# QinLab-WFU/CLIP-based-Cross-Modal-Hashing

Measured on AMD Instinct MI355X. Metric: image+text pairs/s encoded+hashed per GPU; mAP@K eval wallclock (64-bit), higher is better.
Workload: dtype bf16

## Files before the change

### clip-based-cross-modal-hashing_amd/csrc/gemm_lc.hip

```cpp
#include <cstdlib>
#include <cstring>

#include "cmh_common.h"

#include <hip/hip_ext.h>

namespace cmh {

typedef __attribute__((ext_vector_type(8))) __bf16 lc_bf16x8_t;
typedef __attribute__((ext_vector_type(4))) float lc_f32x4_t;
typedef __attribute__((ext_vector_type(2))) float lc_f32x2_t;
typedef __attribute__((ext_vector_type(4))) uint32_t lc_u32x4_t;
typedef __attribute__((ext_vector_type(2))) unsigned lc_u2_t;
typedef const __attribute__((address_space(1))) void* lc_gptr_t;
typedef __attribute__((address_space(3))) void* lc_lptr_t;

constexpr int lcBM = 128, lcBN = 256;
constexpr int lcRowBytes = 128;
constexpr int lcWBytes = lcBN * lcRowBytes;
constexpr int lcSTG = lcWBytes + lcBM * lcRowBytes;

struct LcProblem {
  const char* X; const char* W; const float* bias; const void* residual; void* out;
  const int* m_dev;
  int Mub, N, K;
  const float* colscale = nullptr;
  float alpha = 1.f, oscale = 1.f;
};

__device__ __forceinline__ int lc_swz(int row, int chunk) { return row * lcRowBytes + ((chunk ^ (row & 7)) << 4); }

#define LC_READ(dst, addr, off) asm volatile("ds_read_b128 %0, %1 offset:" #off : "=v"(dst) : "v"(addr))

#ifdef LC_STAMPS
__device__ unsigned long long g_lc_stamps[256 * 8];
#define LC_T() __builtin_amdgcn_s_memtime()
#endif

template <bool GRP, int RES, bool F16O, int ABL = 0>
__global__ __launch_bounds__(512) void gemm_lc_kernel(LcProblem p0, LcProblem p1, int epi) {
  constexpr bool RF = RES == 1;
  __shared__ __attribute__((aligned(1024))) char lds[3 * lcSTG + 2 * 1024];
  const int tid = threadIdx.x;
  const int lane = tid & 63;
  const int wid = __builtin_amdgcn_readfirstlane(tid >> 6);

  const char* const X0 = p0.X; const char* const W0 = p0.W; const float* const B0 = p0.bias;
  const void* const R0 = p0.residual; void* const O0 = p0.out;
  const int N0 = p0.N, K0 = p0.K;
  const char* const X1 = p1.X; const char* const W1 = p1.W; const float* const B1 = p1.bias;
  const void* const R1 = p1.residual; void* const O1 = p1.out;
  const int N1 = p1.N, K1 = p1.K;
  int M0 = p0.Mub;
  if (p0.m_dev) { const int md = *p0.m_dev; M0 = md < M0 ? md : M0; }
  M0 = __builtin_amdgcn_readfirstlane(M0);
  int M1 = 0;
  if constexpr (GRP) {
    M1 = p1.Mub;
    if (p1.m_dev) { const int md = *p1.m_dev; M1 = md < M1 ? md : M1; }
    M1 = __builtin_amdgcn_readfirstlane(M1);
  }
  const int tiles_n0 = N0 / lcBN, tiles_n1 = GRP ? N1 / lcBN : 1;
  const int total0 = tiles_n0 * ((M0 + lcBM - 1) / lcBM);
  const int total1 = GRP ? tiles_n1 * ((M1 + lcBM - 1) / lcBM) : 0;
  const int xcd = blockIdx.x & 7, slot = blockIdx.x >> 3, per = gridDim.x >> 3;
  const int q0 = total0 >> 3, r0 = total0 & 7, q1 = total1 >> 3, r1 = total1 & 7;
  const int lo0 = xcd < r0 ? xcd * (q0 + 1) : r0 * (q0 + 1) + (xcd - r0) * q0, len0 = xcd < r0 ? q0 + 1 : q0;
  const int lo1 = xcd < r1 ? xcd * (q1 + 1) : r1 * (q1 + 1) + (xcd - r1) * q1, len1 = xcd < r1 ? q1 + 1 : q1;
  const int n_first = slot < len0 ? (len0 - slot + per - 1) / per : 0;
  const int span = len0 + len1;
  const int my_tiles = slot < span ? (span - slot + per - 1) / per : 0;
  if (my_tiles == 0) return;
  const int nk0 = K0 / 64, nk1 = GRP ? K1 / 64 : 0;
  const int S = n_first * nk0 + (my_tiles - n_first) * nk1;
  auto tile_of = [&](int ti, bool& second, int& m0, int& n0) {
    const int j = slot + ti * per;
    second = GRP && ti >= n_first;
    const int logical = second ? lo1 + (j - len0) : lo0 + j;
    const int tn_cnt = second ? tiles_n1 : tiles_n0;
    const int tm = logical / tn_cnt;
    m0 = tm * lcBM;
    n0 = (logical - tm * tn_cnt) * lcBN;
  };

  if (wid < 4) {
    const int sub = lane >> 3, ch = lane & 7;
    uint32_t offW[8], offX[4];
    const char* Wt = nullptr;
    const char* Xt = nullptr;
    const char* Bt = nullptr;
    int i_nk = 0;
    int w_prob = -1;
    auto set_tile = [&](int ti) {
      bool second; int m0, n0;
      tile_of(ti, second, m0, n0);
      const uint32_t rs = static_cast<uint32_t>(second ? K1 : K0) * 2;
      if (w_prob != static_cast<int>(second)) {
        w_prob = static_cast<int>(second);
#pragma unroll
        for (int i = 0; i < 8; ++i) {
          const int row = (wid * 8 + i) * 8 + sub;
          offW[i] = static_cast<uint32_t>(row) * rs + ((ch ^ (row & 7)) << 4);
        }
      }
      i_nk = second ? nk1 : nk0;
      const int Mp = second ? M1 : M0;
      Wt = (second ? W1 : W0) + static_cast<size_t>(n0) * rs;
      Xt = second ? X1 : X0;
      Bt = reinterpret_cast<const char*>((second ? B1 : B0) + n0);
#pragma unroll
      for (int i = 0; i < 4; ++i) {
        const int row = (wid * 4 + i) * 8 + sub;
        int xr = m0 + row;
        xr = xr < Mp ? xr : Mp - 1;
        offX[i] = static_cast<uint32_t>(xr) * rs + ((ch ^ (row & 7)) << 4);
      }
    };
    int i_tile = 0, i_kt = 0, ibuf = 0;
    set_tile(0);
    const bool bias_wave = wid == 0 && (epi & EPI_BIAS);
    auto issue_stage = [&]() {
      char* base = lds + ibuf * lcSTG;
      const uint32_t koff = static_cast<uint32_t>(i_kt) * lcRowBytes;
      if (i_kt == 0 && bias_wave)
        __builtin_amdgcn_global_load_lds((lc_gptr_t)(Bt + lane * 16), (lc_lptr_t)(lds + 3 * lcSTG + (i_tile & 1) * 1024), 16, 0, 0);
#pragma unroll
      for (int i = 0; i < 8; ++i)
        __builtin_amdgcn_global_load_lds((lc_gptr_t)(Wt + koff + offW[i]), (lc_lptr_t)(base + (wid * 8 + i) * 1024), 16, 0, 0);
#pragma unroll
      for (int i = 0; i < 4; ++i)
        __builtin_amdgcn_global_load_lds((lc_gptr_t)(Xt + koff + offX[i]), (lc_lptr_t)(base + lcWBytes + (wid * 4 + i) * 1024), 16, 0, 0);
      ibuf = ibuf == 2 ? 0 : ibuf + 1;
      if (++i_kt == i_nk) {
        i_kt = 0;
        if (++i_tile < my_tiles) set_tile(i_tile);
      }
    };
    issue_stage();
    if (S > 1) issue_stage();
    if (S > 2) issue_stage();
    if (S > 2) asm volatile("s_waitcnt vmcnt(24)" ::: "memory");
    else if (S > 1) asm volatile("s_waitcnt vmcnt(12)" ::: "memory");
    else asm volatile("s_waitcnt vmcnt(0)" ::: "memory");
    __builtin_amdgcn_s_barrier();
    for (int s = 0; s < S; ++s) {
      if (s + 2 < S && !(ABL & 4)) asm volatile("s_waitcnt vmcnt(12)" ::: "memory");
      else asm volatile("s_waitcnt vmcnt(0)" ::: "memory");
      __builtin_amdgcn_s_barrier();
      if (s + 3 < S && !(ABL & 2)) issue_stage();
    }
    return;
  }

  const int c = wid - 4;
  const int wm = c >> 1, wn = c & 1;
  const int frow = lane & 15, fq = lane >> 4;
  const uint32_t lds_base = static_cast<uint32_t>(reinterpret_cast<uintptr_t>((lc_lptr_t)lds));
  const uint32_t aW = lds_base + lc_swz(wn * 128 + frow, fq);
  const uint32_t aX = lds_base + lcWBytes + lc_swz(wm * 64 + frow, fq);

  lc_f32x4_t acc[8][4];
  lc_u32x4_t fw[8], fxa[4], fxb[4];

  const void* residual = R0;
  void* out = O0;
  int N = N0, M = M0, nk = nk0;
  [[maybe_unused]] auto to_problem1 = [&]() {
    residual = R1; out = O1; N = N1; M = M1; nk = nk1;
  };
  if constexpr (GRP) { if (n_first == 0) to_problem1(); }

  auto add_residual = [&](int m0, int n0) __attribute__((always_inline)) {
    const uint16_t* res16 = reinterpret_cast<const uint16_t*>(residual);
    const int col = n0 + wn * 128 + (fq & 1) * 16 + (fq & 2) * 4;
#pragma unroll
    for (int bg = 0; bg < 4; bg += 2) {
      lc_u32x4_t r[2][4];
#pragma unroll
      for (int b = bg; b < bg + 2; ++b) {
        int m = m0 + wm * 64 + b * 16 + frow;
        m = m < M ? m : M - 1;
#pragma unroll
        for (int pr = 0; pr < 4; ++pr) r[b - bg][pr] = *reinterpret_cast<const lc_u32x4_t*>(res16 + static_cast<size_t>(m) * N + col + 32 * pr);
      }
#pragma unroll
      for (int b = bg; b < bg + 2; ++b) {
#pragma unroll
        for (int pr = 0; pr < 4; ++pr) {
          const lc_u32x4_t qv = r[b - bg][pr];
          const lc_u2_t s0 = __builtin_amdgcn_permlane16_swap(qv[0], qv[2], false, false);
          const lc_u2_t s1 = __builtin_amdgcn_permlane16_swap(qv[1], qv[3], false, false);
          acc[2 * pr][b][0] += f16lo_to_f32(s0[0]); acc[2 * pr][b][1] += f16hi_to_f32(s0[0]);
          acc[2 * pr][b][2] += f16lo_to_f32(s1[0]); acc[2 * pr][b][3] += f16hi_to_f32(s1[0]);
          acc[2 * pr + 1][b][0] += f16lo_to_f32(s0[1]); acc[2 * pr + 1][b][1] += f16hi_to_f32(s0[1]);
          acc[2 * pr + 1][b][2] += f16lo_to_f32(s1[1]); acc[2 * pr + 1][b][3] += f16hi_to_f32(s1[1]);
        }
      }
    }
  };
  auto zero_acc = [&]() __attribute__((always_inline)) {
#pragma unroll
    for (int a = 0; a < 8; ++a)
#pragma unroll
      for (int b = 0; b < 4; ++b) acc[a][b] = lc_f32x4_t{0.f, 0.f, 0.f, 0.f};
  };
  auto mfma = [&](const lc_u32x4_t& w, const lc_u32x4_t& x, const lc_f32x4_t& cin) __attribute__((always_inline)) {
    if constexpr (ABL & 1) {
      asm volatile("" ::"v"(w), "v"(x));
      return cin;
    } else
    return __builtin_amdgcn_mfma_f32_16x16x32_bf16(__builtin_bit_cast(lc_bf16x8_t, w), __builtin_bit_cast(lc_bf16x8_t, x), cin, 0, 0, 0);
  };
#define LC_WAIT5(cnt, r0, r1, r2, r3, r4) \
  asm volatile("s_waitcnt lgkmcnt(" #cnt ")" : "+v"(r0), "+v"(r1), "+v"(r2), "+v"(r3), "+v"(r4)::"memory")
#define LC_WAIT1(cnt, r0) asm volatile("s_waitcnt lgkmcnt(" #cnt ")" : "+v"(r0)::"memory")
#define LC_WAIT_ALLW(cnt) \
  asm volatile("s_waitcnt lgkmcnt(" #cnt ")" : "+v"(fw[0]), "+v"(fw[1]), "+v"(fw[2]), "+v"(fw[3]), "+v"(fw[4]), "+v"(fw[5]), "+v"(fw[6]), "+v"(fw[7])::"memory")

#define LC_READ_W(a, addr)                                                       \
  do {                                                                           \
    if constexpr ((a) == 0) LC_READ(fw[0], addr, 0);                             \
    else if constexpr ((a) == 1) LC_READ(fw[1], addr, 2048);                     \
    else if constexpr ((a) == 2) LC_READ(fw[2], addr, 4096);                     \
    else if constexpr ((a) == 3) LC_READ(fw[3], addr, 6144);                     \
    else if constexpr ((a) == 4) LC_READ(fw[4], addr, 8192);                     \
    else if constexpr ((a) == 5) LC_READ(fw[5], addr, 10240);                    \
    else if constexpr ((a) == 6) LC_READ(fw[6], addr, 12288);                    \
    else LC_READ(fw[7], addr, 14336);                                            \
  } while (0)
#define LC_READ_X(fx, b, addr)                                                   \
  do {                                                                           \
    if constexpr ((b) == 0) LC_READ(fx[0], addr, 0);                             \
    else if constexpr ((b) == 1) LC_READ(fx[1], addr, 2048);                     \
    else if constexpr ((b) == 2) LC_READ(fx[2], addr, 4096);                     \
    else LC_READ(fx[3], addr, 6144);                                             \
  } while (0)

#ifdef LC_STAMPS
  const unsigned long long st_t0 = LC_T(), st_r0 = __builtin_amdgcn_s_memrealtime();
  unsigned long long st_first = 0, st_k = 0, st_e = 0, st_mark = 0;
#endif
  int cur = 0;
  {
    bool second; int m0, n0;
    tile_of(0, second, m0, n0);
    if constexpr (RF) { zero_acc(); add_residual(m0, n0); }
  }
  __builtin_amdgcn_s_barrier();
#ifdef LC_STAMPS
  st_first = LC_T() - st_t0;
  st_mark = LC_T();
#endif
  LC_READ_X(fxa, 0, aX); LC_READ_X(fxa, 1, aX); LC_READ_X(fxa, 2, aX); LC_READ_X(fxa, 3, aX);
  LC_READ_W(0, aW); LC_READ_W(1, aW); LC_READ_W(2, aW); LC_READ_W(3, aW);
  LC_READ_W(4, aW); LC_READ_W(5, aW); LC_READ_W(6, aW); LC_READ_W(7, aW);

  auto kstep = [&](auto zc) __attribute__((always_inline)) {
    constexpr bool ZC = decltype(zc)::value;
    const uint32_t bo = static_cast<uint32_t>(cur) * lcSTG;
    const uint32_t w1 = (aW + bo) ^ 64u, x1 = (aX + bo) ^ 64u;
    LC_WAIT5(7, fxa[0], fxa[1], fxa[2], fxa[3], fw[0]);
    __builtin_amdgcn_sched_barrier(0);
#define LC_MFMA0(a, b) acc[a][b] = mfma(fw[a], fxa[b], ZC ? lc_f32x4_t{0.f, 0.f, 0.f, 0.f} : acc[a][b])
#define LC_GROUP0(a)                                                                                   \
  do {                                                                                                 \
    if constexpr ((a) > 0) { LC_WAIT1(11, fw[a]); __builtin_amdgcn_sched_barrier(0); }                 \
    if constexpr ((a) == 0) LC_READ_X(fxb, 0, x1);                                                     \
    LC_MFMA0(a, 0);                                                                                    \
    if constexpr ((a) == 0) LC_READ_X(fxb, 1, x1);                                                     \
    LC_MFMA0(a, 1);                                                                                    \
    if constexpr ((a) == 0) LC_READ_X(fxb, 2, x1);                                                     \
    LC_MFMA0(a, 2);                                                                                    \
    if constexpr ((a) == 0) LC_READ_X(fxb, 3, x1);                                                     \
    LC_MFMA0(a, 3);                                                                                    \
    __builtin_amdgcn_sched_barrier(0);                                                                 \
    LC_READ_W(a, w1);                                                                                  \
    __builtin_amdgcn_sched_barrier(0);                                                                 \
  } while (0)
    LC_GROUP0(0); LC_GROUP0(1); LC_GROUP0(2); LC_GROUP0(3); LC_GROUP0(4); LC_GROUP0(5); LC_GROUP0(6); LC_GROUP0(7);
#undef LC_GROUP0
#undef LC_MFMA0
    const int nxt = cur == 2 ? 0 : cur + 1;
    const uint32_t bn = static_cast<uint32_t>(nxt) * lcSTG;
    const uint32_t w0 = aW + bn, x0 = aX + bn;
#define LC_MFMA1(a, b) acc[a][b] = mfma(fw[a], fxb[b], acc[a][b])
    LC_WAIT5(7, fxb[0], fxb[1], fxb[2], fxb[3], fw[0]);
    __builtin_amdgcn_sched_barrier(0);
    LC_MFMA1(0, 0); LC_MFMA1(0, 1); LC_MFMA1(0, 2); LC_MFMA1(0, 3);
    __builtin_amdgcn_sched_barrier(0);
    LC_WAIT1(6, fw[1]);
    __builtin_amdgcn_sched_barrier(0);
    LC_MFMA1(1, 0); LC_MFMA1(1, 1); LC_MFMA1(1, 2); LC_MFMA1(1, 3);
    __builtin_amdgcn_sched_barrier(0);
    LC_WAIT_ALLW(0);
    __builtin_amdgcn_s_barrier();
    __builtin_amdgcn_sched_barrier(0);
    LC_READ_X(fxa, 0, x0);
    LC_MFMA1(2, 0);
    LC_READ_X(fxa, 1, x0);
    LC_MFMA1(2, 1);
    LC_READ_X(fxa, 2, x0);
    LC_MFMA1(2, 2);
    LC_READ_X(fxa, 3, x0);
    LC_MFMA1(2, 3);
    __builtin_amdgcn_sched_barrier(0);
    LC_READ_W(0, w0);
    LC_READ_W(1, w0);
    LC_READ_W(2, w0);
    __builtin_amdgcn_sched_barrier(0);
#define LC_GROUP1(a)                                                                                   \
  do {                                                                                                 \
    LC_MFMA1(a, 0); LC_MFMA1(a, 1); LC_MFMA1(a, 2); LC_MFMA1(a, 3);                                    \
    __builtin_amdgcn_sched_barrier(0);                                                                 \
    LC_READ_W(a, w0);                                                                                  \
    __builtin_amdgcn_sched_barrier(0);                                                                 \
  } while (0)
    LC_GROUP1(3); LC_GROUP1(4); LC_GROUP1(5); LC_GROUP1(6); LC_GROUP1(7);
#undef LC_GROUP1
#undef LC_MFMA1
    cur = nxt;
  };

  for (int ti = 0; ti < my_tiles; ++ti) {
    bool second; int m0, n0;
    tile_of(ti, second, m0, n0);
    if constexpr (GRP) { if (ti == n_first && ti > 0) to_problem1(); }
    if constexpr (RF) { if (ti > 0) { zero_acc(); add_residual(m0, n0); } }
    else zero_acc();
    for (int kt = 0; kt < nk; ++kt) kstep(std::false_type{});

#ifdef LC_STAMPS
    { const unsigned long long t_ = LC_T(); st_k += t_ - st_mark; st_mark = t_; }
#endif
    if (epi & EPI_BIAS) {
      const uint32_t ab = lds_base + 3 * lcSTG + (ti & 1) * 1024 + (wn * 128 + fq * 4) * 4;
      lc_f32x4_t bv[8];
#pragma unroll
      for (int a = 0; a < 8; ++a) asm volatile("ds_read_b128 %0, %1 offset:%2" : "=v"(bv[a]) : "v"(ab), "n"(a * 64));
      asm volatile("s_waitcnt lgkmcnt(0)" : "+v"(bv[0]), "+v"(bv[1]), "+v"(bv[2]), "+v"(bv[3]), "+v"(bv[4]), "+v"(bv[5]), "+v"(bv[6]), "+v"(bv[7])::"memory");
#pragma unroll
      for (int a = 0; a < 8; ++a)
#pragma unroll
        for (int b = 0; b < 4; ++b) acc[a][b] += bv[a];
    }
    if (epi & EPI_QUICKGELU) {
#pragma unroll
      for (int a = 0; a < 8; ++a)
#pragma unroll
        for (int b = 0; b < 4; ++b)
#pragma unroll
          for (int j = 0; j < 4; j += 2) {
            const lc_f32x2_t v = {acc[a][b][j], acc[a][b][j + 1]};
            const lc_f32x2_t t = v * lc_f32x2_t{-2.4554669595930157f, -2.4554669595930157f};
            const lc_f32x2_t d = lc_f32x2_t{__builtin_amdgcn_exp2f(t[0]), __builtin_amdgcn_exp2f(t[1])} + lc_f32x2_t{1.0f, 1.0f};
            const lc_f32x2_t o = v * lc_f32x2_t{__builtin_amdgcn_rcpf(d[0]), __builtin_amdgcn_rcpf(d[1])};
            acc[a][b][j] = o[0];
            acc[a][b][j + 1] = o[1];
          }
    }
    if constexpr (RES == 2) add_residual(m0, n0);
    __builtin_amdgcn_sched_barrier(0);
    {
      char* const obase = static_cast<char*>(out) + (static_cast<size_t>(m0) * N + n0) * 2;
      const uint32_t ldn = static_cast<uint32_t>(N) * 2;
      const uint32_t off0 = static_cast<uint32_t>(wm * 64 + frow) * ldn + static_cast<uint32_t>(wn * 128 + (fq & 1) * 16 + (fq & 2) * 4) * 2;
      const bool full = m0 + lcBM <= M && !(epi & 256);
#pragma unroll
      for (int b = 0; b < 4; ++b) {
        const uint32_t offb = off0 + static_cast<uint32_t>(b * 16) * ldn;
#pragma unroll
        for (int pr = 0; pr < 4; ++pr) {
          uint32_t lo[2], hi[2];
#pragma unroll
          for (int w = 0; w < 2; ++w) {
            if constexpr (F16O) {
              lo[w] = pack_f16x2(acc[2 * pr][b][2 * w], acc[2 * pr][b][2 * w + 1]);
              hi[w] = pack_f16x2(acc[2 * pr + 1][b][2 * w], acc[2 * pr + 1][b][2 * w + 1]);
            } else {
              lo[w] = pack_bf16x2(acc[2 * pr][b][2 * w], acc[2 * pr][b][2 * w + 1]);
              hi[w] = pack_bf16x2(acc[2 * pr + 1][b][2 * w], acc[2 * pr + 1][b][2 * w + 1]);
            }
          }
          const lc_u2_t s0 = __builtin_amdgcn_permlane16_swap(lo[0], hi[0], false, false);
          const lc_u2_t s1 = __builtin_amdgcn_permlane16_swap(lo[1], hi[1], false, false);
          const lc_u32x4_t val = {s0[0], s1[0], s0[1], s1[1]};
          if (full) *reinterpret_cast<lc_u32x4_t*>(obase + (offb + pr * 64)) = val;
          else if (m0 + wm * 64 + b * 16 + frow < M && !(epi & 256)) *reinterpret_cast<lc_u32x4_t*>(obase + (offb + pr * 64)) = val;
        }
      }
    }
#ifdef LC_STAMPS
    { const unsigned long long t_ = LC_T(); st_e += t_ - st_mark; st_mark = t_; }
#endif
  }
#ifdef LC_STAMPS
  if (c == 0 && lane == 0 && blockIdx.x < 256) {
    unsigned long long* o = g_lc_stamps + blockIdx.x * 8;
    o[0] = LC_T() - st_t0; o[1] = __builtin_amdgcn_s_memrealtime() - st_r0; o[2] = st_first; o[3] = st_k; o[4] = st_e;
    o[5] = static_cast<unsigned long long>(S); o[6] = static_cast<unsigned long long>(my_tiles); o[7] = static_cast<unsigned long long>(my_tiles);
  }
#endif
  asm volatile("s_waitcnt lgkmcnt(0)" ::: "memory");
}

template <bool GRP, int RES, bool F16O>
__global__ __launch_bounds__(768) void gemm_lc2_kernel(LcProblem p0, LcProblem p1, int epi) {
  __shared__ __attribute__((aligned(1024))) char lds[3 * lcSTG + 2 * 1024];
  const int tid = threadIdx.x;
  const int lane = tid & 63;
  const int wid = __builtin_amdgcn_readfirstlane(tid >> 6);

  const char* const X0 = p0.X; const char* const W0 = p0.W; const float* const B0 = p0.bias; void* const O0 = p0.out;
  const void* const R0 = p0.residual;
  const int N0 = p0.N, K0 = p0.K;
  const char* const X1 = p1.X; const char* const W1 = p1.W; const float* const B1 = p1.bias; void* const O1 = p1.out;
  const void* const R1 = p1.residual;
  const int N1 = p1.N, K1 = p1.K;
  int M0 = p0.Mub;
  if (p0.m_dev) { const int md = *p0.m_dev; M0 = md < M0 ? md : M0; }
  M0 = __builtin_amdgcn_readfirstlane(M0);
  int M1 = 0;
  if constexpr (GRP) {
    M1 = p1.Mub;
    if (p1.m_dev) { const int md = *p1.m_dev; M1 = md < M1 ? md : M1; }
    M1 = __builtin_amdgcn_readfirstlane(M1);
  }
  const int tiles_n0 = N0 / lcBN, tiles_n1 = GRP ? N1 / lcBN : 1;
  const int total0 = tiles_n0 * ((M0 + lcBM - 1) / lcBM);
  const int total1 = GRP ? tiles_n1 * ((M1 + lcBM - 1) / lcBM) : 0;
  const int xcd = blockIdx.x & 7, slot = blockIdx.x >> 3, per = gridDim.x >> 3;
  const int q0 = total0 >> 3, r0 = total0 & 7, q1 = total1 >> 3, r1 = total1 & 7;
  const int lo0 = xcd < r0 ? xcd * (q0 + 1) : r0 * (q0 + 1) + (xcd - r0) * q0, len0 = xcd < r0 ? q0 + 1 : q0;
  const int lo1 = xcd < r1 ? xcd * (q1 + 1) : r1 * (q1 + 1) + (xcd - r1) * q1, len1 = xcd < r1 ? q1 + 1 : q1;
  const int n_first = slot < len0 ? (len0 - slot + per - 1) / per : 0;
  const int span = len0 + len1;
  const int my_tiles = slot < span ? (span - slot + per - 1) / per : 0;
  if (my_tiles == 0) return;
  const int nk0 = K0 / 64, nk1 = GRP ? K1 / 64 : 0;
  const int S = n_first * nk0 + (my_tiles - n_first) * nk1;
  auto tile_of = [&](int ti, bool& second, int& m0, int& n0) {
    const int j = slot + ti * per;
    second = GRP && ti >= n_first;
    const int logical = second ? lo1 + (j - len0) : lo0 + j;
    const int tn_cnt = second ? tiles_n1 : tiles_n0;
    const int tm = logical / tn_cnt;
    m0 = tm * lcBM;
    n0 = (logical - tm * tn_cnt) * lcBN;
  };

  if (wid < 4) {
    const int sub = lane >> 3, ch = lane & 7;
    uint32_t offW[8], offX[4];
    const char* Wt = nullptr;
    const char* Xt = nullptr;
    const char* Bt = nullptr;
    int i_nk = 0;
    int w_prob = -1;
    auto set_tile = [&](int ti) {
      bool second; int m0, n0;
      tile_of(ti, second, m0, n0);
      const uint32_t rs = static_cast<uint32_t>(second ? K1 : K0) * 2;
      if (w_prob != static_cast<int>(second)) {
        w_prob = static_cast<int>(second);
#pragma unroll
        for (int i = 0; i < 8; ++i) {
          const int row = (wid * 8 + i) * 8 + sub;
          offW[i] = static_cast<uint32_t>(row) * rs + ((ch ^ (row & 7)) << 4);
        }
      }
      i_nk = second ? nk1 : nk0;
      const int Mp = second ? M1 : M0;
      Wt = (second ? W1 : W0) + static_cast<size_t>(n0) * rs;
      Xt = second ? X1 : X0;
      Bt = reinterpret_cast<const char*>((second ? B1 : B0) + n0);
#pragma unroll
      for (int i = 0; i < 4; ++i) {
        const int row = (wid * 4 + i) * 8 + sub;
        int xr = m0 + row;
        xr = xr < Mp ? xr : Mp - 1;
        offX[i] = static_cast<uint32_t>(xr) * rs + ((ch ^ (row & 7)) << 4);
      }
    };
    int i_tile = 0, i_kt = 0, ibuf = 0;
    set_tile(0);
    const bool bias_wave = wid == 0 && (epi & EPI_BIAS);
    auto issue_stage = [&]() {
      char* base = lds + ibuf * lcSTG;
      const uint32_t koff = static_cast<uint32_t>(i_kt) * lcRowBytes;
      if (i_kt == 0 && bias_wave)
        __builtin_amdgcn_global_load_lds((lc_gptr_t)(Bt + lane * 16), (lc_lptr_t)(lds + 3 * lcSTG + (i_tile & 1) * 1024), 16, 0, 0);
#pragma unroll
      for (int i = 0; i < 8; ++i)
        __builtin_amdgcn_global_load_lds((lc_gptr_t)(Wt + koff + offW[i]), (lc_lptr_t)(base + (wid * 8 + i) * 1024), 16, 0, 0);
#pragma unroll
      for (int i = 0; i < 4; ++i)
        __builtin_amdgcn_global_load_lds((lc_gptr_t)(Xt + koff + offX[i]), (lc_lptr_t)(base + lcWBytes + (wid * 4 + i) * 1024), 16, 0, 0);
      ibuf = ibuf == 2 ? 0 : ibuf + 1;
      if (++i_kt == i_nk) {
        i_kt = 0;
        if (++i_tile < my_tiles) set_tile(i_tile);
      }
    };
    issue_stage();
    if (S > 1) issue_stage();
    if (S > 2) issue_stage();
    if (S > 2) asm volatile("s_waitcnt vmcnt(24)" ::: "memory");
    else if (S > 1) asm volatile("s_waitcnt vmcnt(12)" ::: "memory");
    else asm volatile("s_waitcnt vmcnt(0)" ::: "memory");
    __builtin_amdgcn_s_barrier();
    for (int s = 0; s < S; ++s) {
      if (s + 2 < S) asm volatile("s_waitcnt vmcnt(12)" ::: "memory");
      else asm volatile("s_waitcnt vmcnt(0)" ::: "memory");
      __builtin_amdgcn_s_barrier();
      if (s + 3 < S) issue_stage();
    }
    return;
  }

  const int c = wid - 4;
  const int wm = c >> 2, wn = c & 3;
  const int frow = lane & 15, fq = lane >> 4;
  const uint32_t lds_base = static_cast<uint32_t>(reinterpret_cast<uintptr_t>((lc_lptr_t)lds));
  const uint32_t aW = lds_base + lc_swz(wn * 64 + frow, fq);
  const uint32_t aX = lds_base + lcWBytes + lc_swz(wm * 64 + frow, fq);

  lc_f32x4_t acc[4][4];
  lc_u32x4_t fw[4], fxa[4], fxb[4];
  lc_u32x4_t pend[8];
  int pend_idx = 8;
  char* pend_base = nullptr;
  uint32_t pend_off0 = 0, pend_ldn = 0;
  [[maybe_unused]] int res_kt = -1, res_tile = -1;

  void* out = O0;
  int N = N0, M = M0, nk = nk0;
  [[maybe_unused]] auto to_problem1 = [&]() { out = O1; N = N1; M = M1; nk = nk1; };
  if constexpr (GRP) { if (n_first == 0) to_problem1(); }

  auto mfma = [&](const lc_u32x4_t& w, const lc_u32x4_t& x, const lc_f32x4_t& cin) __attribute__((always_inline)) {
    return __builtin_amdgcn_mfma_f32_16x16x32_bf16(__builtin_bit_cast(lc_bf16x8_t, w), __builtin_bit_cast(lc_bf16x8_t, x), cin, 0, 0, 0);
  };
  auto store_pending = [&](int idx) __attribute__((always_inline)) {
    char* p = pend_base + (pend_off0 + static_cast<uint32_t>(idx >> 1) * 16u * pend_ldn + static_cast<uint32_t>(idx & 1) * 64u);
    switch (idx) {
      case 0: *reinterpret_cast<lc_u32x4_t*>(p) = pend[0]; break;
      case 1: *reinterpret_cast<lc_u32x4_t*>(p) = pend[1]; break;
      case 2: *reinterpret_cast<lc_u32x4_t*>(p) = pend[2]; break;
      case 3: *reinterpret_cast<lc_u32x4_t*>(p) = pend[3]; break;
      case 4: *reinterpret_cast<lc_u32x4_t*>(p) = pend[4]; break;
      case 5: *reinterpret_cast<lc_u32x4_t*>(p) = pend[5]; break;
      case 6: *reinterpret_cast<lc_u32x4_t*>(p) = pend[6]; break;
      default: *reinterpret_cast<lc_u32x4_t*>(p) = pend[7]; break;
    }
  };
  [[maybe_unused]] auto fetch_residual = [&](int ti) __attribute__((always_inline)) {
    bool second; int m0, n0;
    tile_of(ti, second, m0, n0);
    const uint16_t* res16 = reinterpret_cast<const uint16_t*>(second ? R1 : R0);
    const int Nn = second ? N1 : N0, Mp = second ? M1 : M0;
    const int col = n0 + wn * 64 + (fq & 1) * 16 + (fq & 2) * 4;
#pragma unroll
    for (int b = 0; b < 4; ++b) {
      int m = m0 + wm * 64 + b * 16 + frow;
      m = m < Mp ? m : Mp - 1;
#pragma unroll
      for (int pr = 0; pr < 2; ++pr) pend[2 * b + pr] = *reinterpret_cast<const lc_u32x4_t*>(res16 + static_cast<size_t>(m) * Nn + col + 32 * pr);
    }
  };
  [[maybe_unused]] auto add_piece = [&](int b, int pr, const lc_u32x4_t& qv) __attribute__((always_inline)) {
    const lc_u2_t s0 = __builtin_amdgcn_permlane16_swap(qv[0], qv[2], false, false);
    const lc_u2_t s1 = __builtin_amdgcn_permlane16_swap(qv[1], qv[3], false, false);
    acc[2 * pr][b][0] += f16lo_to_f32(s0[0]); acc[2 * pr][b][1] += f16hi_to_f32(s0[0]);
    acc[2 * pr][b][2] += f16lo_to_f32(s1[0]); acc[2 * pr][b][3] += f16hi_to_f32(s1[0]);
    acc[2 * pr + 1][b][0] += f16lo_to_f32(s0[1]); acc[2 * pr + 1][b][1] += f16hi_to_f32(s0[1]);
    acc[2 * pr + 1][b][2] += f16lo_to_f32(s1[1]); acc[2 * pr + 1][b][3] += f16hi_to_f32(s1[1]);
  };
#define L2_WAIT5(cnt, r0, r1, r2, r3, r4) \
  asm volatile("s_waitcnt lgkmcnt(" #cnt ")" : "+v"(r0), "+v"(r1), "+v"(r2), "+v"(r3), "+v"(r4)::"memory")
#define L2_WAIT1(cnt, r0) asm volatile("s_waitcnt lgkmcnt(" #cnt ")" : "+v"(r0)::"memory")
#define L2_WAIT_ALLW(cnt) asm volatile("s_waitcnt lgkmcnt(" #cnt ")" : "+v"(fw[0]), "+v"(fw[1]), "+v"(fw[2]), "+v"(fw[3])::"memory")
#define L2_READ_W(a, addr)                                                       \
  do {                                                                           \
    if constexpr ((a) == 0) LC_READ(fw[0], addr, 0);                             \
    else if constexpr ((a) == 1) LC_READ(fw[1], addr, 2048);                     \
    else if constexpr ((a) == 2) LC_READ(fw[2], addr, 4096);                     \
    else LC_READ(fw[3], addr, 6144);                                             \
  } while (0)
#define L2_READ_X(fx, b, addr)                                                   \
  do {                                                                           \
    if constexpr ((b) == 0) LC_READ(fx[0], addr, 0);                             \
    else if constexpr ((b) == 1) LC_READ(fx[1], addr, 2048);                     \
    else if constexpr ((b) == 2) LC_READ(fx[2], addr, 4096);                     \
    else LC_READ(fx[3], addr, 6144);                                             \
  } while (0)

  int cur = 0;
  if constexpr (RES == 1) {
    fetch_residual(0);
#pragma unroll
    for (int a = 0; a < 4; ++a)
#pragma unroll
      for (int b = 0; b < 4; ++b) acc[a][b] = lc_f32x4_t{0.f, 0.f, 0.f, 0.f};
#pragma unroll
    for (int b = 0; b < 4; ++b)
#pragma unroll
      for (int pr = 0; pr < 2; ++pr) add_piece(b, pr, pend[2 * b + pr]);
  }
  __builtin_amdgcn_s_barrier();
  L2_READ_X(fxa, 0, aX); L2_READ_X(fxa, 1, aX); L2_READ_X(fxa, 2, aX); L2_READ_X(fxa, 3, aX);
  L2_READ_W(0, aW); L2_READ_W(1, aW); L2_READ_W(2, aW); L2_READ_W(3, aW);

  auto kstep = [&](int kt) __attribute__((always_inline)) {
    const uint32_t bo = static_cast<uint32_t>(cur) * lcSTG;
    const uint32_t w1 = (aW + bo) ^ 64u, x1 = (aX + bo) ^ 64u;
    L2_WAIT5(3, fxa[0], fxa[1], fxa[2], fxa[3], fw[0]);
    __builtin_amdgcn_sched_barrier(0);
#define L2_MFMA0(a, b) acc[a][b] = mfma(fw[a], fxa[b], acc[a][b])
#define L2_GROUP0(a)                                                                                   \
  do {                                                                                                 \
    if constexpr ((a) > 0) { L2_WAIT1(7, fw[a]); __builtin_amdgcn_sched_barrier(0); }                  \
    if constexpr ((a) == 0) L2_READ_X(fxb, 0, x1);                                                     \
    L2_MFMA0(a, 0);                                                                                    \
    if constexpr ((a) == 0) L2_READ_X(fxb, 1, x1);                                                     \
    L2_MFMA0(a, 1);                                                                                    \
    if constexpr ((a) == 0) L2_READ_X(fxb, 2, x1);                                                     \
    L2_MFMA0(a, 2);                                                                                    \
    if constexpr ((a) == 0) L2_READ_X(fxb, 3, x1);                                                     \
    L2_MFMA0(a, 3);                                                                                    \
    __builtin_amdgcn_sched_barrier(0);                                                                 \
    L2_READ_W(a, w1);                                                                                  \
    __builtin_amdgcn_sched_barrier(0);                                                                 \
  } while (0)
    L2_GROUP0(0); L2_GROUP0(1);
    if (pend_idx < 8) {
      store_pending(pend_idx); store_pending(pend_idx + 1);
      pend_idx += 2;
      asm volatile("" : "+s"(pend_idx));
      __builtin_amdgcn_sched_barrier(0);
    }
    if constexpr (RES != 0) {
      if (kt == res_kt) { fetch_residual(res_tile); __builtin_amdgcn_sched_barrier(0); }
    }
    L2_GROUP0(2); L2_GROUP0(3);
#undef L2_GROUP0
#undef L2_MFMA0
    const int nxt = cur == 2 ? 0 : cur + 1;
    const uint32_t bn = static_cast<uint32_t>(nxt) * lcSTG;
    const uint32_t w0 = aW + bn, x0 = aX + bn;
#define L2_MFMA1(a, b) acc[a][b] = mfma(fw[a], fxb[b], acc[a][b])
    L2_WAIT5(3, fxb[0], fxb[1], fxb[2], fxb[3], fw[0]);
    __builtin_amdgcn_sched_barrier(0);
    L2_MFMA1(0, 0); L2_MFMA1(0, 1); L2_MFMA1(0, 2); L2_MFMA1(0, 3);
    __builtin_amdgcn_sched_barrier(0);
    L2_WAIT1(2, fw[1]);
    __builtin_amdgcn_sched_barrier(0);
    L2_MFMA1(1, 0); L2_MFMA1(1, 1); L2_MFMA1(1, 2); L2_MFMA1(1, 3);
    __builtin_amdgcn_sched_barrier(0);
    L2_WAIT_ALLW(0);
    __builtin_amdgcn_s_barrier();
    __builtin_amdgcn_sched_barrier(0);
    L2_READ_X(fxa, 0, x0);
    L2_MFMA1(2, 0);
    L2_READ_X(fxa, 1, x0);
    L2_MFMA1(2, 1);
    L2_READ_X(fxa, 2, x0);
    L2_MFMA1(2, 2);
    L2_READ_X(fxa, 3, x0);
    L2_MFMA1(2, 3);
    __builtin_amdgcn_sched_barrier(0);
    L2_READ_W(0, w0);
    L2_READ_W(1, w0);
    L2_READ_W(2, w0);
    __builtin_amdgcn_sched_barrier(0);
    L2_MFMA1(3, 0); L2_MFMA1(3, 1); L2_MFMA1(3, 2); L2_MFMA1(3, 3);
    __builtin_amdgcn_sched_barrier(0);
    L2_READ_W(3, w0);
    __builtin_amdgcn_sched_barrier(0);
#undef L2_MFMA1
    cur = nxt;
  };

  for (int ti = 0; ti < my_tiles; ++ti) {
    bool second; int m0, n0;
    tile_of(ti, second, m0, n0);
    if constexpr (GRP) { if (ti == n_first && ti > 0) to_problem1(); }
    if constexpr (RES != 1) {
#pragma unroll
      for (int a = 0; a < 4; ++a)
#pragma unroll
        for (int b = 0; b < 4; ++b) acc[a][b] = lc_f32x4_t{0.f, 0.f, 0.f, 0.f};
    }
    if constexpr (RES == 1) { res_tile = ti + 1; res_kt = ti + 1 < my_tiles ? 4 : -1; }
    if constexpr (RES == 2) { res_tile = ti; res_kt = 4; }
    if constexpr (RES != 0) asm volatile("" : "+s"(res_kt));
    for (int kt = 0; kt < nk; ++kt) {
      asm volatile("" : "+s"(kt));
      kstep(kt);
    }

    if (epi & EPI_BIAS) {
      const uint32_t ab = lds_base + 3 * lcSTG + (ti & 1) * 1024 + (wn * 64 + fq * 4) * 4;
      lc_f32x4_t bv[4];
#pragma unroll
      for (int a = 0; a < 4; ++a) asm volatile("ds_read_b128 %0, %1 offset:%2" : "=v"(bv[a]) : "v"(ab), "n"(a * 64));
      asm volatile("s_waitcnt lgkmcnt(0)" : "+v"(bv[0]), "+v"(bv[1]), "+v"(bv[2]), "+v"(bv[3])::"memory");
#pragma unroll
      for (int a = 0; a < 4; ++a)
#pragma unroll
        for (int b = 0; b < 4; ++b) acc[a][b] += bv[a];
    }
    if (epi & EPI_QUICKGELU) {
#pragma unroll
      for (int a = 0; a < 4; ++a)
#pragma unroll
        for (int b = 0; b < 4; ++b)
#pragma unroll
          for (int j = 0; j < 4; j += 2) {
            const lc_f32x2_t v = {acc[a][b][j], acc[a][b][j + 1]};
            const lc_f32x2_t t = v * lc_f32x2_t{-2.4554669595930157f, -2.4554669595930157f};
            const lc_f32x2_t d = lc_f32x2_t{__builtin_amdgcn_exp2f(t[0]), __builtin_amdgcn_exp2f(t[1])} + lc_f32x2_t{1.0f, 1.0f};
            const lc_f32x2_t o = v * lc_f32x2_t{__builtin_amdgcn_rcpf(d[0]), __builtin_amdgcn_rcpf(d[1])};
            acc[a][b][j] = o[0];
            acc[a][b][j + 1] = o[1];
          }
    }
    if constexpr (RES == 2) {
      asm volatile("s_waitcnt vmcnt(0)" : "+v"(pend[0]), "+v"(pend[1]), "+v"(pend[2]), "+v"(pend[3]), "+v"(pend[4]), "+v"(pend[5]), "+v"(pend[6]), "+v"(pend[7])::"memory");
#pragma unroll
      for (int b = 0; b < 4; ++b)
#pragma unroll
        for (int pr = 0; pr < 2; ++pr) add_piece(b, pr, pend[2 * b + pr]);
    }
    if constexpr (RES == 1) {
      if (res_kt >= 0)
        asm volatile("s_waitcnt vmcnt(0)" : "+v"(pend[0]), "+v"(pend[1]), "+v"(pend[2]), "+v"(pend[3]), "+v"(pend[4]), "+v"(pend[5]), "+v"(pend[6]), "+v"(pend[7])::"memory");
    }
    __builtin_amdgcn_sched_barrier(0);
    {
      char* const obase = static_cast<char*>(out) + (static_cast<size_t>(m0) * N + n0) * 2;
      const uint32_t ldn = static_cast<uint32_t>(N) * 2;
      const uint32_t off0 = static_cast<uint32_t>(wm * 64 + frow) * ldn + static_cast<uint32_t>(wn * 64 + (fq & 1) * 16 + (fq & 2) * 4) * 2;
#pragma unroll
      for (int b = 0; b < 4; ++b)
#pragma unroll
        for (int pr = 0; pr < 2; ++pr) {
          uint32_t lo[2], hi[2];
#pragma unroll
          for (int w = 0; w < 2; ++w) {
            if constexpr (F16O) {
              lo[w] = pack_f16x2(acc[2 * pr][b][2 * w], acc[2 * pr][b][2 * w + 1]);
              hi[w] = pack_f16x2(acc[2 * pr + 1][b][2 * w], acc[2 * pr + 1][b][2 * w + 1]);
            } else {
              lo[w] = pack_bf16x2(acc[2 * pr][b][2 * w], acc[2 * pr][b][2 * w + 1]);
              hi[w] = pack_bf16x2(acc[2 * pr + 1][b][2 * w], acc[2 * pr + 1][b][2 * w + 1]);
            }
          }
          const lc_u2_t s0 = __builtin_amdgcn_permlane16_swap(lo[0], hi[0], false, false);
          const lc_u2_t s1 = __builtin_amdgcn_permlane16_swap(lo[1], hi[1], false, false);
          if constexpr (RES == 1) {
            const lc_u32x4_t nextres = pend[2 * b + pr];
            acc[2 * pr][b] = lc_f32x4_t{0.f, 0.f, 0.f, 0.f};
            acc[2 * pr + 1][b] = lc_f32x4_t{0.f, 0.f, 0.f, 0.f};
            if (res_kt >= 0) add_piece(b, pr, nextres);
          }
          pend[2 * b + pr] = lc_u32x4_t{s0[0], s1[0], s0[1], s1[1]};
        }
      pend_base = obase; pend_off0 = off0; pend_ldn = ldn;
      const bool full = m0 + lcBM <= M;
      if (full && ti + 1 < my_tiles && !(epi & 256)) {
        pend_idx = 0;
        asm volatile("" : "+s"(pend_idx));
      } else if (!(epi & 256)) {
#pragma unroll
        for (int b = 0; b < 4; ++b)
#pragma unroll
          for (int pr = 0; pr < 2; ++pr)
            if (m0 + wm * 64 + b * 16 + frow < M)
              *reinterpret_cast<lc_u32x4_t*>(obase + (off0 + static_cast<uint32_t>(b * 16) * ldn + pr * 64)) = pend[2 * b + pr];
      }
    }
  }
  asm volatile("s_waitcnt lgkmcnt(0)" ::: "memory");
#undef L2_WAIT5
#undef L2_WAIT1
#undef L2_WAIT_ALLW
#undef L2_READ_W
#undef L2_READ_X
}

int gemm_lc_mode();
template <bool GRP>
__global__ __launch_bounds__(768) void gemm_lc2q_kernel(LcProblem p0, LcProblem p1, int epi) {
  static_assert(!GRP, "first form: plain launches");
  __shared__ __attribute__((aligned(1024))) char lds[3 * lcSTG];
  const int tid = threadIdx.x;
  const int lane = tid & 63;
  const int wid = __builtin_amdgcn_readfirstlane(tid >> 6);
  const char* const X0 = p0.X; const char* const W0 = p0.W; const float* const B0 = p0.bias; void* const O0 = p0.out;
  const float* const CS0 = p0.colscale; const float alpha0 = p0.alpha;
  const int N0 = p0.N, K0 = p0.K;
  int M0 = p0.Mub;
  if (p0.m_dev) { const int md = *p0.m_dev; M0 = md < M0 ? md : M0; }
  M0 = __builtin_amdgcn_readfirstlane(M0);
  const int tiles_n0 = N0 / lcBN;
  const int total0 = tiles_n0 * ((M0 + lcBM - 1) / lcBM);
  const int xcd = blockIdx.x & 7, slot = blockIdx.x >> 3, per = gridDim.x >> 3;
  const int q0 = total0 >> 3, r0 = total0 & 7;
  const int lo0 = xcd < r0 ? xcd * (q0 + 1) : r0 * (q0 + 1) + (xcd - r0) * q0, len0 = xcd < r0 ? q0 + 1 : q0;
  const int my_tiles = slot < len0 ? (len0 - slot + per - 1) / per : 0;
  if (my_tiles == 0) return;
  const int nk0 = K0 / 128;
  const int S = my_tiles * nk0;
  auto tile_of = [&](int ti, int& m0, int& n0) {
    const int logical = lo0 + slot + ti * per;
    const int tm = logical / tiles_n0;
    m0 = tm * lcBM;
    n0 = (logical - tm * tiles_n0) * lcBN;
  };
  if (wid < 4) {
    const int sub = lane >> 3, ch = lane & 7;
    uint32_t offW[8], offX[4];
    const char* Wt = nullptr;
    const uint32_t rs = static_cast<uint32_t>(K0);
#pragma unroll
    for (int i = 0; i < 8; ++i) {
      const int row = (wid * 8 + i) * 8 + sub;
      offW[i] = static_cast<uint32_t>(row) * rs + ((ch ^ (row & 7)) << 4);
    }
    auto set_tile = [&](int ti) {
      int m0, n0;
      tile_of(ti, m0, n0);
      Wt = W0 + static_cast<size_t>(n0) * rs;
#pragma unroll
      for (int i = 0; i < 4; ++i) {
        const int row = (wid * 4 + i) * 8 + sub;
        int xr = m0 + row;
        xr = xr < M0 ? xr : M0 - 1;
        offX[i] = static_cast<uint32_t>(xr) * rs + ((ch ^ (row & 7)) << 4);
      }
    };
    int i_tile = 0, i_kt = 0, ibuf = 0;
    set_tile(0);
    auto issue_stage = [&]() {
      char* base = lds + ibuf * lcSTG;
      const uint32_t koff = static_cast<uint32_t>(i_kt) * lcRowBytes;
#pragma unroll
      for (int i = 0; i < 8; ++i)
        __builtin_amdgcn_global_load_lds((lc_gptr_t)(Wt + koff + offW[i]), (lc_lptr_t)(base + (wid * 8 + i) * 1024), 16, 0, 0);
#pragma unroll
      for (int i = 0; i < 4; ++i)
        __builtin_amdgcn_global_load_lds((lc_gptr_t)(X0 + koff + offX[i]), (lc_lptr_t)(base + lcWBytes + (wid * 4 + i) * 1024), 16, 0, 0);
      ibuf = ibuf == 2 ? 0 : ibuf + 1;
      if (++i_kt == nk0) {
        i_kt = 0;
        if (++i_tile < my_tiles) set_tile(i_tile);
      }
    };
    issue_stage();
    if (S > 1) issue_stage();
    if (S > 2) issue_stage();
    if (S > 2) asm volatile("s_waitcnt vmcnt(24)" ::: "memory");
    else if (S > 1) asm volatile("s_waitcnt vmcnt(12)" ::: "memory");
    else asm volatile("s_waitcnt vmcnt(0)" ::: "memory");
    __builtin_amdgcn_s_barrier();
    for (int s = 0; s < S; ++s) {
      if (s + 2 < S) asm volatile("s_waitcnt vmcnt(12)" ::: "memory");
      else asm volatile("s_waitcnt vmcnt(0)" ::: "memory");
      __builtin_amdgcn_s_barrier();
      if (s + 3 < S) issue_stage();
    }
    return;
  }
  const int c = wid - 4;
  const int wm = c >> 2, wn = c & 3;
  const int frow = lane & 15, fq = lane >> 4;
  const uint32_t lds_base = static_cast<uint32_t>(reinterpret_cast<uintptr_t>((lc_lptr_t)lds));
  const uint32_t aW = lds_base + lc_swz(wn * 64 + frow, fq);
  const uint32_t aX = lds_base + lcWBytes + lc_swz(wm * 64 + frow, fq);
  typedef __attribute__((ext_vector_type(8))) int lc_i32x8_t;
  lc_f32x4_t acc[4][4];
  lc_u32x4_t fw[4][2], fx[4][2];
  lc_u32x4_t pend[4];
  int pend_idx = 4;
  char* pend_base = nullptr;
  uint32_t pend_off0 = 0, pend_ldn = 0;
  auto store_pending = [&](int idx) __attribute__((always_inline)) {
    char* p = pend_base + (pend_off0 + static_cast<uint32_t>(2 + (idx >> 1)) * 16u * pend_ldn + static_cast<uint32_t>(idx & 1) * 64u);
    switch (idx) {
      case 0: *reinterpret_cast<lc_u32x4_t*>(p) = pend[0]; break;
      case 1: *reinterpret_cast<lc_u32x4_t*>(p) = pend[1]; break;
      case 2: *reinterpret_cast<lc_u32x4_t*>(p) = pend[2]; break;
      default: *reinterpret_cast<lc_u32x4_t*>(p) = pend[3]; break;
    }
  };
  auto mfma8 = [&](int a, int b) __attribute__((always_inline)) {
    lc_i32x8_t va, vb;
#pragma unroll
    for (int j = 0; j < 4; ++j) {
      va[j] = static_cast<int>(fw[a][0][j]); va[4 + j] = static_cast<int>(fw[a][1][j]);
      vb[j] = static_cast<int>(fx[b][0][j]); vb[4 + j] = static_cast<int>(fx[b][1][j]);
    }
    acc[a][b] = __builtin_amdgcn_mfma_scale_f32_16x16x128_f8f6f4(va, vb, acc[a][b], 0, 0, 0, 0x7f7f7f7f, 0, 0x7f7f7f7f);
  };
#define Q_READ2(dst, addr, off)                                                                                   \
  do {                                                                                                            \
    asm volatile("ds_read_b128 %0, %1 offset:%2" : "=v"(dst[0]) : "v"(addr), "n"(off));                          \
    asm volatile("ds_read_b128 %0, %1 offset:%2" : "=v"(dst[1]) : "v"((addr) ^ 64u), "n"(off));                  \
  } while (0)
#define Q_WAIT_ALL()                                                                                               \
  asm volatile("s_waitcnt lgkmcnt(0)"                                                                             \
               : "+v"(fw[0][0]), "+v"(fw[0][1]), "+v"(fw[1][0]), "+v"(fw[1][1]), "+v"(fw[2][0]), "+v"(fw[2][1]), "+v"(fw[3][0]), "+v"(fw[3][1]), \
                 "+v"(fx[0][0]), "+v"(fx[0][1]), "+v"(fx[1][0]), "+v"(fx[1][1]), "+v"(fx[2][0]), "+v"(fx[2][1]), "+v"(fx[3][0]), "+v"(fx[3][1])::"memory")
  int cur = 0;
  __builtin_amdgcn_s_barrier();
  Q_READ2(fx[0], aX, 0); Q_READ2(fx[1], aX, 2048); Q_READ2(fx[2], aX, 4096); Q_READ2(fx[3], aX, 6144);
  Q_READ2(fw[0], aW, 0); Q_READ2(fw[1], aW, 2048); Q_READ2(fw[2], aW, 4096); Q_READ2(fw[3], aW, 6144);
  auto kstep = [&]() __attribute__((always_inline)) {
    Q_WAIT_ALL();
    __builtin_amdgcn_s_barrier();
    __builtin_amdgcn_sched_barrier(0);
    const int nxt = cur == 2 ? 0 : cur + 1;
    const uint32_t bn = static_cast<uint32_t>(nxt) * lcSTG;
    const uint32_t w0 = aW + bn, x0 = aX + bn;
    mfma8(0, 0); mfma8(0, 1); mfma8(0, 2); mfma8(0, 3);
    __builtin_amdgcn_sched_barrier(0);
    Q_READ2(fw[0], w0, 0);
    __builtin_amdgcn_sched_barrier(0);
    mfma8(1, 0); mfma8(1, 1); mfma8(1, 2); mfma8(1, 3);
    __builtin_amdgcn_sched_barrier(0);
    if (pend_idx < 4) {
      store_pending(pend_idx); store_pending(pend_idx + 1);
      pend_idx += 2;
      asm volatile("" : "+s"(pend_idx));
      __builtin_amdgcn_sched_barrier(0);
    }
    Q_READ2(fw[1], w0, 2048);
    __builtin_amdgcn_sched_barrier(0);
    mfma8(2, 0); mfma8(2, 1); mfma8(2, 2); mfma8(2, 3);
    __builtin_amdgcn_sched_barrier(0);
    Q_READ2(fw[2], w0, 4096);
    __builtin_amdgcn_sched_barrier(0);
    mfma8(3, 0);
    __builtin_amdgcn_sched_barrier(0);
    Q_READ2(fx[0], x0, 0);
    __builtin_amdgcn_sched_barrier(0);
    mfma8(3, 1);
    __builtin_amdgcn_sched_barrier(0);
    Q_READ2(fx[1], x0, 2048);
    __builtin_amdgcn_sched_barrier(0);
    mfma8(3, 2);
    __builtin_amdgcn_sched_barrier(0);
    Q_READ2(fx[2], x0, 4096);
    __builtin_amdgcn_sched_barrier(0);
    mfma8(3, 3);
    __builtin_amdgcn_sched_barrier(0);
    Q_READ2(fx[3], x0, 6144);
    Q_READ2(fw[3], w0, 6144);
    __builtin_amdgcn_sched_barrier(0);
    cur = nxt;
  };
  for (int ti = 0; ti < my_tiles; ++ti) {
    int m0, n0;
    tile_of(ti, m0, n0);
#pragma unroll
    for (int a = 0; a < 4; ++a)
#pragma unroll
      for (int b = 0; b < 4; ++b) acc[a][b] = lc_f32x4_t{0.f, 0.f, 0.f, 0.f};
    for (int kt = 0; kt < nk0; ++kt) kstep();
#pragma unroll
    for (int a = 0; a < 4; ++a) {
      const lc_f32x4_t cs = *reinterpret_cast<const lc_f32x4_t*>(CS0 + n0 + wn * 64 + a * 16 + fq * 4) * alpha0;
      const lc_f32x4_t bv = (epi & EPI_BIAS) ? *reinterpret_cast<const lc_f32x4_t*>(B0 + n0 + wn * 64 + a * 16 + fq * 4) : lc_f32x4_t{0.f, 0.f, 0.f, 0.f};
#pragma unroll
      for (int b = 0; b < 4; ++b) acc[a][b] = acc[a][b] * cs + bv;
    }
    char* const obase = static_cast<char*>(O0) + (static_cast<size_t>(m0) * N0 + n0) * 2;
    const uint32_t ldn = static_cast<uint32_t>(N0) * 2;
    const uint32_t off0 = static_cast<uint32_t>(wm * 64 + frow) * ldn + static_cast<uint32_t>(wn * 64 + (fq & 1) * 16 + (fq & 2) * 4) * 2;
    const bool park = m0 + lcBM <= M0 && ti + 1 < my_tiles && !(epi & 256);
#pragma unroll
    for (int b = 0; b < 4; ++b)
#pragma unroll
      for (int pr = 0; pr < 2; ++pr) {
        uint32_t lo[2], hi[2];
#pragma unroll
        for (int w = 0; w < 2; ++w) {
          lo[w] = pack_bf16x2(acc[2 * pr][b][2 * w], acc[2 * pr][b][2 * w + 1]);
          hi[w] = pack_bf16x2(acc[2 * pr + 1][b][2 * w], acc[2 * pr + 1][b][2 * w + 1]);
        }
        const lc_u2_t s0 = __builtin_amdgcn_permlane16_swap(lo[0], hi[0], false, false);
        const lc_u2_t s1 = __builtin_amdgcn_permlane16_swap(lo[1], hi[1], false, false);
        const lc_u32x4_t val = {s0[0], s1[0], s0[1], s1[1]};
        if (b >= 2) pend[(b - 2) * 2 + pr] = val;
        if ((b < 2 || !park) && m0 + wm * 64 + b * 16 + frow < M0 && !(epi & 256))
          *reinterpret_cast<lc_u32x4_t*>(obase + (off0 + static_cast<uint32_t>(b * 16) * ldn + pr * 64)) = val;
      }
    if (park) {
      pend_base = obase; pend_off0 = off0; pend_ldn = ldn;
      pend_idx = 0;
      asm volatile("" : "+s"(pend_idx));
    }
  }
  asm volatile("s_waitcnt lgkmcnt(0)" ::: "memory");
#undef Q_READ2
#undef Q_WAIT_ALL
}

int launch_gemm_lc2q(const GemmProblem& g, int epi, hipStream_t st, hipEvent_t ev0, hipEvent_t ev1) {
  if (static_cast<size_t>(g.M) * g.K >= (1ull << 32)) return fail(CMH_ERR_INVALID, "gemm (lc2q): operand exceeds the 32-bit offset range");
  LcProblem P0{static_cast<const char*>(g.A), static_cast<const char*>(g.W), g.bias, g.residual, g.out, g.m_dev, g.M, g.N, g.K};
  P0.colscale = g.colscale; P0.alpha = g.alpha; P0.oscale = g.oscale;
  const LcProblem P1{};
  const int total = (g.N / lcBN) * ((g.M + lcBM - 1) / lcBM);
  int cus = 256;
  { int dev = 0; hipDeviceProp_t prop; if (hipGetDevice(&dev) == hipSuccess && hipGetDeviceProperties(&prop, dev) == hipSuccess && prop.multiProcessorCount >= 8) cus = prop.multiProcessorCount & ~7; }
  const int grid = total < cus ? ((total + 7) & ~7) : cus;
  if (ev0) hipExtLaunchKernelGGL((gemm_lc2q_kernel<false>), dim3(grid), dim3(768), 0, st, ev0, ev1, 0, P0, P1, epi);
  else hipLaunchKernelGGL((gemm_lc2q_kernel<false>), dim3(grid), dim3(768), 0, st, P0, P1, epi);
  CMH_CHECK_LAUNCH("gemm (lc2q)");
  return 0;
}
bool gemm_lc2q_takes(int N, int K, int epi) {
  return gemm_lc_mode() == 7 && N % lcBN == 0 && K % 128 == 0 && K >= 512 &&
         (epi & ~(EPI_BIAS | EPI_SCALE | 256)) == EPI_OUT_BF16;
}

static int lc_env_mode() { static const int m = []() { const char* e = getenv("CMH_GEMM_LC"); return e ? atoi(e) : 0; }(); return m; }
static int g_lc_mode = -1;
int gemm_lc_mode() { return g_lc_mode < 0 ? lc_env_mode() : g_lc_mode; }
void gemm_lc_set_mode(int m) { g_lc_mode = m; }

bool gemm_lc_takes(int dt, int N, int K, int epi) {
  if (dt != CMH_BF16 || N % lcBN != 0 || K % 64 != 0 || K < 256) return false;
  if (gemm_lc_mode() >= 4) {
    if (K < 512) return false;
    if (gemm_lc_mode() >= 5 && (epi & EPI_QUICKGELU)) return false;
    if (gemm_lc_mode() == 6 && (epi & EPI_RESIDUAL) && K / 64 > 16) return false;
  }
  if (!(epi & (EPI_OUT_BF16 | EPI_OUT_F16)) || ((epi & EPI_OUT_BF16) && (epi & EPI_OUT_F16))) return false;
  if (epi & ~(EPI_BIAS | EPI_QUICKGELU | EPI_RESIDUAL | EPI_RES_F16 | EPI_OUT_BF16 | EPI_OUT_F16 | 256)) return false;
  if ((epi & EPI_RESIDUAL) && !((epi & EPI_RES_F16) && (epi & EPI_OUT_F16))) return false;
  if ((epi & EPI_RESIDUAL) && (epi & EPI_QUICKGELU)) return false;
  return true;
}

bool gemm_lc_res_first(int epi, int K) {
  return (epi & EPI_RESIDUAL) && !(epi & (EPI_QUICKGELU | EPI_GELU | EPI_RELU)) && K / 64 <= 16;
}

static int lc_cus() {
  static int cus = 0;
  if (!cus) {
    int dev = 0;
    hipDeviceProp_t prop;
    if (hipGetDevice(&dev) == hipSuccess && hipGetDeviceProperties(&prop, dev) == hipSuccess) cus = prop.multiProcessorCount;
    if (cus < 8) cus = 256;
    cus &= ~7;
  }
  return cus;
}

int launch_gemm_lc(const GemmProblem& a, const GemmProblem* b, int epi, hipStream_t st, hipEvent_t ev0, hipEvent_t ev1) {
  for (const GemmProblem* g : {&a, b}) {
    if (!g) continue;
    if (static_cast<size_t>(g->M) * g->K * 2 >= (1ull << 32) || static_cast<size_t>(lcBN) * g->K * 2 >= (1ull << 32))
      return fail(CMH_ERR_INVALID, "gemm (lc): operand of %zu bytes exceeds the 32-bit offset range", static_cast<size_t>(g->M) * g->K * 2);
  }
  auto prob = [](const GemmProblem& g) {
    return LcProblem{static_cast<const char*>(g.A), static_cast<const char*>(g.W), g.bias, g.residual, g.out, g.m_dev, g.M, g.N, g.K};
  };
  auto tiles_of = [](const GemmProblem& g) { return (g.N / lcBN) * ((g.M + lcBM - 1) / lcBM); };
  const int cus = lc_cus();
  const int total = tiles_of(a) + (b ? tiles_of(*b) : 0);
  const int grid = total < cus ? ((total + 7) & ~7) : cus;
  const LcProblem P0 = prob(a), P1 = b ? prob(*b) : LcProblem{};
  if (gemm_lc_mode() >= 4) {
    const int res2 = !(epi & EPI_RESIDUAL) ? 0 : (gemm_lc_res_first(epi, a.K) ? 1 : 2);
    const bool f16 = (epi & EPI_OUT_F16) != 0;
#define LC2_GO(G, R, F)                                                                                                       \
  do {                                                                                                                       \
    if (ev0) hipExtLaunchKernelGGL((gemm_lc2_kernel<G, R, F>), dim3(grid), dim3(768), 0, st, ev0, ev1, 0, P0, P1, epi);      \
    else hipLaunchKernelGGL((gemm_lc2_kernel<G, R, F>), dim3(grid), dim3(768), 0, st, P0, P1, epi);                          \
  } while (0)
#define LC2_GO_G(G)                                                                                                           \
  do {                                                                                                                       \
    if (res2 == 1) LC2_GO(G, 1, true);                                                                                       \
    else if (res2 == 2) LC2_GO(G, 2, true);                                                                                  \
    else if (f16) LC2_GO(G, 0, true);                                                                                        \
    else LC2_GO(G, 0, false);                                                                                                \
  } while (0)
    if (b) LC2_GO_G(true); else LC2_GO_G(false);
#undef LC2_GO_G
#undef LC2_GO
    CMH_CHECK_LAUNCH("gemm (lc2)");
    return 0;
  }
  const bool rf = gemm_lc_res_first(epi, a.K);
  const bool f16o = (epi & EPI_OUT_F16) != 0;
#define LC_GO2(G, R, F)                                                                                                      \
  do {                                                                                                                       \
    if (ev0) hipExtLaunchKernelGGL((gemm_lc_kernel<G, R, F>), dim3(grid), dim3(512), 0, st, ev0, ev1, 0, P0, P1, epi);       \
    else hipLaunchKernelGGL((gemm_lc_kernel<G, R, F>), dim3(grid), dim3(512), 0, st, P0, P1, epi);                           \
  } while (0)
  const int res = !(epi & EPI_RESIDUAL) ? 0 : (rf ? 1 : 2);
#define LC_GO(G, R_unused)                                                                                                   \
  do {                                                                                                                       \
    if (res == 1) LC_GO2(G, 1, true);                                                                                        \
    else if (res == 2) LC_GO2(G, 2, true);                                                                                   \
    else if (f16o) LC_GO2(G, 0, true);                                                                                       \
    else LC_GO2(G, 0, false);                                                                                                \
  } while (0)
  static const int abl = []() { const char* e = getenv("CMH_LC_ABL"); return e ? atoi(e) : 0; }();
  if (abl && !b && !rf && !(epi & EPI_OUT_F16)) {
#define LC_GO_A(A)                                                                                                            \
  do {                                                                                                                       \
    if (ev0) hipExtLaunchKernelGGL((gemm_lc_kernel<false, 0, false, A>), dim3(grid), dim3(512), 0, st, ev0, ev1, 0, P0, P1, epi); \
    else hipLaunchKernelGGL((gemm_lc_kernel<false, 0, false, A>), dim3(grid), dim3(512), 0, st, P0, P1, epi);                    \
  } while (0)
    if (abl == 1) LC_GO_A(1); else if (abl == 2) LC_GO_A(2); else if (abl == 3) LC_GO_A(3); else LC_GO_A(4);
#undef LC_GO_A
    CMH_CHECK_LAUNCH("gemm (lc, diagnostic)");
    return 0;
  }
  if (b) { if (rf) LC_GO(true, true); else LC_GO(true, false); }
  else { if (rf) LC_GO(false, true); else LC_GO(false, false); }
#undef LC_GO
#undef LC_GO2
  CMH_CHECK_LAUNCH("gemm (lc)");
  return 0;
}

}

#ifdef LC_STAMPS
extern "C" int cmh_debug_lc_stamps(unsigned long long* host_out) {
  return hipMemcpyFromSymbol(host_out, HIP_SYMBOL(cmh::g_lc_stamps), sizeof(unsigned long long) * 256 * 8) == hipSuccess ? 0 : -1;
}
#endif

extern "C" int cmh_set_gemm_lc(int32_t mode) {
  CMH_CHECK_ARG(mode >= -1 && mode <= 7, "set_gemm_lc: mode %d (-1 environment, 0 off, 1 every eligible launch, 2 all but QuickGELU launches, 3 by cost model, 4 / 5 / 6 the 12-wave form for every block launch / without the QuickGELU ones / for QKV and out_proj only)", mode);
  cmh::gemm_lc_set_mode(mode);
  return CMH_OK;
}
```

Baseline: 59950.

## Add 160-row tile variant to 12-wave GEMM and enable it by default for QKV

Templates the 12-wave LDS-staged GEMM on the number of M fragments so it can run 160-row tiles (5 MFMA fragments per wave). The extra fragment adds a new k-step schedule and adjusted vmcnt thresholds, and the default mode becomes 9, which routes non-residual, non-QuickGELU launches through this kernel. Hand-written ds_read asm and explicit lgkmcnt waits are replaced with volatile LDS loads, leaving the compiler to place the waits. The larger tile aims for more reuse of each W fragment and fewer tiles, at the cost of more registers and LDS, a different occupancy, and possibly poorer tile quantisation for some M.

```diff
diff --git a/clip-based-cross-modal-hashing_amd/csrc/gemm_lc.hip b/clip-based-cross-modal-hashing_amd/csrc/gemm_lc.hip
--- a/clip-based-cross-modal-hashing_amd/csrc/gemm_lc.hip
+++ b/clip-based-cross-modal-hashing_amd/csrc/gemm_lc.hip
@@ -30,7 +30,17 @@
 
 __device__ __forceinline__ int lc_swz(int row, int chunk) { return row * lcRowBytes + ((chunk ^ (row & 7)) << 4); }
 
-#define LC_READ(dst, addr, off) asm volatile("ds_read_b128 %0, %1 offset:" #off : "=v"(dst) : "v"(addr))
+__device__ __forceinline__ lc_u32x4_t lc_lds_read(uint32_t addr) {
+  return *reinterpret_cast<volatile __attribute__((address_space(3))) lc_u32x4_t*>(static_cast<uintptr_t>(addr));
+}
+#define LC_READ(dst, addr, off) ((dst) = lc_lds_read((addr) + (off)))
+#define LC_DRAIN() asm volatile("s_waitcnt lgkmcnt(0)" ::: "memory")
+#define LC_BARRIER()                          \
+  do {                                        \
+    asm volatile("" ::: "memory");            \
+    __builtin_amdgcn_s_barrier();             \
+    asm volatile("" ::: "memory");            \
+  } while (0)
 
 #ifdef LC_STAMPS
 __device__ unsigned long long g_lc_stamps[256 * 8];
@@ -211,11 +221,6 @@
     } else
     return __builtin_amdgcn_mfma_f32_16x16x32_bf16(__builtin_bit_cast(lc_bf16x8_t, w), __builtin_bit_cast(lc_bf16x8_t, x), cin, 0, 0, 0);
   };
-#define LC_WAIT5(cnt, r0, r1, r2, r3, r4) \
-  asm volatile("s_waitcnt lgkmcnt(" #cnt ")" : "+v"(r0), "+v"(r1), "+v"(r2), "+v"(r3), "+v"(r4)::"memory")
-#define LC_WAIT1(cnt, r0) asm volatile("s_waitcnt lgkmcnt(" #cnt ")" : "+v"(r0)::"memory")
-#define LC_WAIT_ALLW(cnt) \
-  asm volatile("s_waitcnt lgkmcnt(" #cnt ")" : "+v"(fw[0]), "+v"(fw[1]), "+v"(fw[2]), "+v"(fw[3]), "+v"(fw[4]), "+v"(fw[5]), "+v"(fw[6]), "+v"(fw[7])::"memory")
 
 #define LC_READ_W(a, addr)                                                       \
   do {                                                                           \
@@ -246,7 +251,7 @@
     tile_of(0, second, m0, n0);
     if constexpr (RF) { zero_acc(); add_residual(m0, n0); }
   }
-  __builtin_amdgcn_s_barrier();
+  LC_BARRIER();
 #ifdef LC_STAMPS
   st_first = LC_T() - st_t0;
   st_mark = LC_T();
@@ -259,12 +264,9 @@
     constexpr bool ZC = decltype(zc)::value;
     const uint32_t bo = static_cast<uint32_t>(cur) * lcSTG;
     const uint32_t w1 = (aW + bo) ^ 64u, x1 = (aX + bo) ^ 64u;
-    LC_WAIT5(7, fxa[0], fxa[1], fxa[2], fxa[3], fw[0]);
-    __builtin_amdgcn_sched_barrier(0);
 #define LC_MFMA0(a, b) acc[a][b] = mfma(fw[a], fxa[b], ZC ? lc_f32x4_t{0.f, 0.f, 0.f, 0.f} : acc[a][b])
 #define LC_GROUP0(a)                                                                                   \
   do {                                                                                                 \
-    if constexpr ((a) > 0) { LC_WAIT1(11, fw[a]); __builtin_amdgcn_sched_barrier(0); }                 \
     if constexpr ((a) == 0) LC_READ_X(fxb, 0, x1);                                                     \
     LC_MFMA0(a, 0);                                                                                    \
     if constexpr ((a) == 0) LC_READ_X(fxb, 1, x1);                                                     \
@@ -284,16 +286,12 @@
     const uint32_t bn = static_cast<uint32_t>(nxt) * lcSTG;
     const uint32_t w0 = aW + bn, x0 = aX + bn;
 #define LC_MFMA1(a, b) acc[a][b] = mfma(fw[a], fxb[b], acc[a][b])
-    LC_WAIT5(7, fxb[0], fxb[1], fxb[2], fxb[3], fw[0]);
-    __builtin_amdgcn_sched_barrier(0);
     LC_MFMA1(0, 0); LC_MFMA1(0, 1); LC_MFMA1(0, 2); LC_MFMA1(0, 3);
     __builtin_amdgcn_sched_barrier(0);
-    LC_WAIT1(6, fw[1]);
-    __builtin_amdgcn_sched_barrier(0);
     LC_MFMA1(1, 0); LC_MFMA1(1, 1); LC_MFMA1(1, 2); LC_MFMA1(1, 3);
     __builtin_amdgcn_sched_barrier(0);
-    LC_WAIT_ALLW(0);
-    __builtin_amdgcn_s_barrier();
+    LC_DRAIN();
+    LC_BARRIER();
     __builtin_amdgcn_sched_barrier(0);
     LC_READ_X(fxa, 0, x0);
     LC_MFMA1(2, 0);
@@ -336,8 +334,7 @@
       const uint32_t ab = lds_base + 3 * lcSTG + (ti & 1) * 1024 + (wn * 128 + fq * 4) * 4;
       lc_f32x4_t bv[8];
 #pragma unroll
-      for (int a = 0; a < 8; ++a) asm volatile("ds_read_b128 %0, %1 offset:%2" : "=v"(bv[a]) : "v"(ab), "n"(a * 64));
-      asm volatile("s_waitcnt lgkmcnt(0)" : "+v"(bv[0]), "+v"(bv[1]), "+v"(bv[2]), "+v"(bv[3]), "+v"(bv[4]), "+v"(bv[5]), "+v"(bv[6]), "+v"(bv[7])::"memory");
+      for (int a = 0; a < 8; ++a) bv[a] = __builtin_bit_cast(lc_f32x4_t, lc_lds_read(ab + a * 64));
 #pragma unroll
       for (int a = 0; a < 8; ++a)
 #pragma unroll
@@ -403,9 +400,13 @@
   asm volatile("s_waitcnt lgkmcnt(0)" ::: "memory");
 }
 
-template <bool GRP, int RES, bool F16O>
+template <int MF, bool GRP, int RES, bool F16O>
 __global__ __launch_bounds__(768) void gemm_lc2_kernel(LcProblem p0, LcProblem p1, int epi) {
-  __shared__ __attribute__((aligned(1024))) char lds[3 * lcSTG + 2 * 1024];
+  static_assert(MF == 4 || MF == 5, "128- or 160-row tiles");
+  constexpr int BM = 32 * MF;
+  constexpr int STG = lcWBytes + BM * lcRowBytes;
+  constexpr int NP = 2 * MF;
+  __shared__ __attribute__((aligned(1024))) char lds[3 * STG + 2 * 1024];
   const int tid = threadIdx.x;
   const int lane = tid & 63;
   const int wid = __builtin_amdgcn_readfirstlane(tid >> 6);
@@ -426,8 +427,8 @@
     M1 = __builtin_amdgcn_readfirstlane(M1);
   }
   const int tiles_n0 = N0 / lcBN, tiles_n1 = GRP ? N1 / lcBN : 1;
-  const int total0 = tiles_n0 * ((M0 + lcBM - 1) / lcBM);
-  const int total1 = GRP ? tiles_n1 * ((M1 + lcBM - 1) / lcBM) : 0;
+  const int total0 = tiles_n0 * ((M0 + BM - 1) / BM);
+  const int total1 = GRP ? tiles_n1 * ((M1 + BM - 1) / BM) : 0;
   const int xcd = blockIdx.x & 7, slot = blockIdx.x >> 3, per = gridDim.x >> 3;
   const int q0 = total0 >> 3, r0 = total0 & 7, q1 = total1 >> 3, r1 = total1 & 7;
   const int lo0 = xcd < r0 ? xcd * (q0 + 1) : r0 * (q0 + 1) + (xcd - r0) * q0, len0 = xcd < r0 ? q0 + 1 : q0;
@@ -444,13 +445,13 @@
     const int logical = second ? lo1 + (j - len0) : lo0 + j;
     const int tn_cnt = second ? tiles_n1 : tiles_n0;
     const int tm = logical / tn_cnt;
-    m0 = tm * lcBM;
+    m0 = tm * BM;
     n0 = (logical - tm * tn_cnt) * lcBN;
   };
 
   if (wid < 4) {
     const int sub = lane >> 3, ch = lane & 7;
-    uint32_t offW[8], offX[4];
+    uint32_t offW[8], offX[MF];
     const char* Wt = nullptr;
     const char* Xt = nullptr;
     const char* Bt = nullptr;
@@ -474,8 +475,8 @@
       Xt = second ? X1 : X0;
       Bt = reinterpret_cast<const char*>((second ? B1 : B0) + n0);
 #pragma unroll
-      for (int i = 0; i < 4; ++i) {
-        const int row = (wid * 4 + i) * 8 + sub;
+      for (int i = 0; i < MF; ++i) {
+        const int row = (wid * MF + i) * 8 + sub;
         int xr = m0 + row;
         xr = xr < Mp ? xr : Mp - 1;
         offX[i] = static_cast<uint32_t>(xr) * rs + ((ch ^ (row & 7)) << 4);
@@ -485,16 +486,16 @@
     set_tile(0);
     const bool bias_wave = wid == 0 && (epi & EPI_BIAS);
     auto issue_stage = [&]() {
-      char* base = lds + ibuf * lcSTG;
+      char* base = lds + ibuf * STG;
       const uint32_t koff = static_cast<uint32_t>(i_kt) * lcRowBytes;
       if (i_kt == 0 && bias_wave)
-        __builtin_amdgcn_global_load_lds((lc_gptr_t)(Bt + lane * 16), (lc_lptr_t)(lds + 3 * lcSTG + (i_tile & 1) * 1024), 16, 0, 0);
+        __builtin_amdgcn_global_load_lds((lc_gptr_t)(Bt + lane * 16), (lc_lptr_t)(lds + 3 * STG + (i_tile & 1) * 1024), 16, 0, 0);
 #pragma unroll
       for (int i = 0; i < 8; ++i)
         __builtin_amdgcn_global_load_lds((lc_gptr_t)(Wt + koff + offW[i]), (lc_lptr_t)(base + (wid * 8 + i) * 1024), 16, 0, 0);
 #pragma unroll
-      for (int i = 0; i < 4; ++i)
-        __builtin_amdgcn_global_load_lds((lc_gptr_t)(Xt + koff + offX[i]), (lc_lptr_t)(base + lcWBytes + (wid * 4 + i) * 1024), 16, 0, 0);
+      for (int i = 0; i < MF; ++i)
+        __builtin_amdgcn_global_load_lds((lc_gptr_t)(Xt + koff + offX[i]), (lc_lptr_t)(base + lcWBytes + (wid * MF + i) * 1024), 16, 0, 0);
       ibuf = ibuf == 2 ? 0 : ibuf + 1;
       if (++i_kt == i_nk) {
         i_kt = 0;
@@ -504,12 +505,12 @@
     issue_stage();
     if (S > 1) issue_stage();
     if (S > 2) issue_stage();
-    if (S > 2) asm volatile("s_waitcnt vmcnt(24)" ::: "memory");
-    else if (S > 1) asm volatile("s_waitcnt vmcnt(12)" ::: "memory");
+    if (S > 2) { if constexpr (MF == 5) asm volatile("s_waitcnt vmcnt(26)" ::: "memory"); else asm volatile("s_waitcnt vmcnt(24)" ::: "memory"); }
+    else if (S > 1) { if constexpr (MF == 5) asm volatile("s_waitcnt vmcnt(13)" ::: "memory"); else asm volatile("s_waitcnt vmcnt(12)" ::: "memory"); }
     else asm volatile("s_waitcnt vmcnt(0)" ::: "memory");
     __builtin_amdgcn_s_barrier();
     for (int s = 0; s < S; ++s) {
-      if (s + 2 < S) asm volatile("s_waitcnt vmcnt(12)" ::: "memory");
+      if (s + 2 < S) { if constexpr (MF == 5) asm volatile("s_waitcnt vmcnt(13)" ::: "memory"); else asm volatile("s_waitcnt vmcnt(12)" ::: "memory"); }
       else asm volatile("s_waitcnt vmcnt(0)" ::: "memory");
       __builtin_amdgcn_s_barrier();
       if (s + 3 < S) issue_stage();
@@ -522,12 +523,12 @@
   const int frow = lane & 15, fq = lane >> 4;
   const uint32_t lds_base = static_cast<uint32_t>(reinterpret_cast<uintptr_t>((lc_lptr_t)lds));
   const uint32_t aW = lds_base + lc_swz(wn * 64 + frow, fq);
-  const uint32_t aX = lds_base + lcWBytes + lc_swz(wm * 64 + frow, fq);
-
-  lc_f32x4_t acc[4][4];
-  lc_u32x4_t fw[4], fxa[4], fxb[4];
-  lc_u32x4_t pend[8];
-  int pend_idx = 8;
+  const uint32_t aX = lds_base + lcWBytes + lc_swz(wm * 16 * MF + frow, fq);
+
+  lc_f32x4_t acc[4][MF];
+  lc_u32x4_t fw[4], fxa[MF], fxb[MF];
+  lc_u32x4_t pend[NP];
+  int pend_idx = NP;
   char* pend_base = nullptr;
   uint32_t pend_off0 = 0, pend_ldn = 0;
   [[maybe_unused]] int res_kt = -1, res_tile = -1;
@@ -550,7 +551,9 @@
       case 4: *reinterpret_cast<lc_u32x4_t*>(p) = pend[4]; break;
       case 5: *reinterpret_cast<lc_u32x4_t*>(p) = pend[5]; break;
       case 6: *reinterpret_cast<lc_u32x4_t*>(p) = pend[6]; break;
-      default: *reinterpret_cast<lc_u32x4_t*>(p) = pend[7]; break;
+      case 7: *reinterpret_cast<lc_u32x4_t*>(p) = pend[7]; break;
+      case 8: if constexpr (NP > 8) *reinterpret_cast<lc_u32x4_t*>(p) = pend[8]; break;
+      default: if constexpr (NP > 9) *reinterpret_cast<lc_u32x4_t*>(p) = pend[9]; break;
     }
   };
   [[maybe_unused]] auto fetch_residual = [&](int ti) __attribute__((always_inline)) {
@@ -560,8 +563,8 @@
     const int Nn = second ? N1 : N0, Mp = second ? M1 : M0;
     const int col = n0 + wn * 64 + (fq & 1) * 16 + (fq & 2) * 4;
 #pragma unroll
-    for (int b = 0; b < 4; ++b) {
-      int m = m0 + wm * 64 + b * 16 + frow;
+    for (int b = 0; b < MF; ++b) {
+      int m = m0 + wm * 16 * MF + b * 16 + frow;
       m = m < Mp ? m : Mp - 1;
 #pragma unroll
       for (int pr = 0; pr < 2; ++pr) pend[2 * b + pr] = *reinterpret_cast<const lc_u32x4_t*>(res16 + static_cast<size_t>(m) * Nn + col + 32 * pr);
@@ -575,24 +578,13 @@
     acc[2 * pr + 1][b][0] += f16lo_to_f32(s0[1]); acc[2 * pr + 1][b][1] += f16hi_to_f32(s0[1]);
     acc[2 * pr + 1][b][2] += f16lo_to_f32(s1[1]); acc[2 * pr + 1][b][3] += f16hi_to_f32(s1[1]);
   };
-#define L2_WAIT5(cnt, r0, r1, r2, r3, r4) \
-  asm volatile("s_waitcnt lgkmcnt(" #cnt ")" : "+v"(r0), "+v"(r1), "+v"(r2), "+v"(r3), "+v"(r4)::"memory")
-#define L2_WAIT1(cnt, r0) asm volatile("s_waitcnt lgkmcnt(" #cnt ")" : "+v"(r0)::"memory")
-#define L2_WAIT_ALLW(cnt) asm volatile("s_waitcnt lgkmcnt(" #cnt ")" : "+v"(fw[0]), "+v"(fw[1]), "+v"(fw[2]), "+v"(fw[3])::"memory")
-#define L2_READ_W(a, addr)                                                       \
-  do {                                                                           \
-    if constexpr ((a) == 0) LC_READ(fw[0], addr, 0);                             \
-    else if constexpr ((a) == 1) LC_READ(fw[1], addr, 2048);                     \
-    else if constexpr ((a) == 2) LC_READ(fw[2], addr, 4096);                     \
-    else LC_READ(fw[3], addr, 6144);                                             \
-  } while (0)
-#define L2_READ_X(fx, b, addr)                                                   \
-  do {                                                                           \
-    if constexpr ((b) == 0) LC_READ(fx[0], addr, 0);                             \
-    else if constexpr ((b) == 1) LC_READ(fx[1], addr, 2048);                     \
-    else if constexpr ((b) == 2) LC_READ(fx[2], addr, 4096);                     \
-    else LC_READ(fx[3], addr, 6144);                                             \
-  } while (0)
+#define L2_PEND_WAIT()                                                                                                                \
+  do {                                                                                                                              \
+    asm volatile("s_waitcnt vmcnt(0)" : "+v"(pend[0]), "+v"(pend[1]), "+v"(pend[2]), "+v"(pend[3]), "+v"(pend[4]), "+v"(pend[5]), "+v"(pend[6]), "+v"(pend[7])::"memory"); \
+    if constexpr (NP > 8) asm volatile("" : "+v"(pend[NP > 8 ? 8 : 0]), "+v"(pend[NP > 9 ? 9 : 0]));                                    \
+  } while (0)
+#define L2_READ_W(a, addr) LC_READ(fw[a], addr, (a) * 2048)
+#define L2_READ_X(fx, b, addr) LC_READ(fx[b], addr, (b) * 2048)
 
   int cur = 0;
   if constexpr (RES == 1) {
@@ -600,25 +592,23 @@
 #pragma unroll
     for (int a = 0; a < 4; ++a)
 #pragma unroll
-      for (int b = 0; b < 4; ++b) acc[a][b] = lc_f32x4_t{0.f, 0.f, 0.f, 0.f};
-#pragma unroll
-    for (int b = 0; b < 4; ++b)
+      for (int b = 0; b < MF; ++b) acc[a][b] = lc_f32x4_t{0.f, 0.f, 0.f, 0.f};
+#pragma unroll
+    for (int b = 0; b < MF; ++b)
 #pragma unroll
       for (int pr = 0; pr < 2; ++pr) add_piece(b, pr, pend[2 * b + pr]);
   }
-  __builtin_amdgcn_s_barrier();
+  LC_BARRIER();
   L2_READ_X(fxa, 0, aX); L2_READ_X(fxa, 1, aX); L2_READ_X(fxa, 2, aX); L2_READ_X(fxa, 3, aX);
+  if constexpr (MF == 5) L2_READ_X(fxa, 4, aX);
   L2_READ_W(0, aW); L2_READ_W(1, aW); L2_READ_W(2, aW); L2_READ_W(3, aW);
 
   auto kstep = [&](int kt) __attribute__((always_inline)) {
-    const uint32_t bo = static_cast<uint32_t>(cur) * lcSTG;
+    const uint32_t bo = static_cast<uint32_t>(cur) * STG;
     const uint32_t w1 = (aW + bo) ^ 64u, x1 = (aX + bo) ^ 64u;
-    L2_WAIT5(3, fxa[0], fxa[1], fxa[2], fxa[3], fw[0]);
-    __builtin_amdgcn_sched_barrier(0);
 #define L2_MFMA0(a, b) acc[a][b] = mfma(fw[a], fxa[b], acc[a][b])
 #define L2_GROUP0(a)                                                                                   \
   do {                                                                                                 \
-    if constexpr ((a) > 0) { L2_WAIT1(7, fw[a]); __builtin_amdgcn_sched_barrier(0); }                  \
     if constexpr ((a) == 0) L2_READ_X(fxb, 0, x1);                                                     \
     L2_MFMA0(a, 0);                                                                                    \
     if constexpr ((a) == 0) L2_READ_X(fxb, 1, x1);                                                     \
@@ -632,7 +622,7 @@
     __builtin_amdgcn_sched_barrier(0);                                                                 \
   } while (0)
     L2_GROUP0(0); L2_GROUP0(1);
-    if (pend_idx < 8) {
+    if (pend_idx < NP) {
       store_pending(pend_idx); store_pending(pend_idx + 1);
       pend_idx += 2;
       asm volatile("" : "+s"(pend_idx));
@@ -645,19 +635,15 @@
 #undef L2_GROUP0
 #undef L2_MFMA0
     const int nxt = cur == 2 ? 0 : cur + 1;
-    const uint32_t bn = static_cast<uint32_t>(nxt) * lcSTG;
+    const uint32_t bn = static_cast<uint32_t>(nxt) * STG;
     const uint32_t w0 = aW + bn, x0 = aX + bn;
 #define L2_MFMA1(a, b) acc[a][b] = mfma(fw[a], fxb[b], acc[a][b])
-    L2_WAIT5(3, fxb[0], fxb[1], fxb[2], fxb[3], fw[0]);
-    __builtin_amdgcn_sched_barrier(0);
     L2_MFMA1(0, 0); L2_MFMA1(0, 1); L2_MFMA1(0, 2); L2_MFMA1(0, 3);
     __builtin_amdgcn_sched_barrier(0);
-    L2_WAIT1(2, fw[1]);
-    __builtin_amdgcn_sched_barrier(0);
     L2_MFMA1(1, 0); L2_MFMA1(1, 1); L2_MFMA1(1, 2); L2_MFMA1(1, 3);
     __builtin_amdgcn_sched_barrier(0);
-    L2_WAIT_ALLW(0);
-    __builtin_amdgcn_s_barrier();
+    LC_DRAIN();
+    LC_BARRIER();
     __builtin_amdgcn_sched_barrier(0);
     L2_READ_X(fxa, 0, x0);
     L2_MFMA1(2, 0);
@@ -679,6 +665,59 @@
 #undef L2_MFMA1
     cur = nxt;
   };
+  [[maybe_unused]] auto kstep5 = [&](int kt) __attribute__((always_inline)) {
+    if constexpr (MF == 5) {
+    const uint32_t bo = static_cast<uint32_t>(cur) * STG;
+    const uint32_t w1 = (aW + bo) ^ 64u, x1 = (aX + bo) ^ 64u;
+#define L5_MFMAS(a)                                                                                    \
+  do {                                                                                                 \
+    acc[a][0] = mfma(fw[a], fxa[0], acc[a][0]); acc[a][1] = mfma(fw[a], fxa[1], acc[a][1]);            \
+    acc[a][2] = mfma(fw[a], fxa[2], acc[a][2]); acc[a][3] = mfma(fw[a], fxa[3], acc[a][3]);            \
+    acc[a][4] = mfma(fw[a], fxa[4], acc[a][4]);                                                        \
+    __builtin_amdgcn_sched_barrier(0);                                                                 \
+  } while (0)
+#define L5_LAST(xaddr, waddr)                                                                          \
+  do {                                                                                                 \
+    acc[3][0] = mfma(fw[3], fxa[0], acc[3][0]); __builtin_amdgcn_sched_barrier(0);                     \
+    L2_READ_X(fxa, 0, xaddr); __builtin_amdgcn_sched_barrier(0);                                       \
+    acc[3][1] = mfma(fw[3], fxa[1], acc[3][1]); __builtin_amdgcn_sched_barrier(0);                     \
+    L2_READ_X(fxa, 1, xaddr); __builtin_amdgcn_sched_barrier(0);                                       \
+    acc[3][2] = mfma(fw[3], fxa[2], acc[3][2]); __builtin_amdgcn_sched_barrier(0);                     \
+    L2_READ_X(fxa, 2, xaddr); __builtin_amdgcn_sched_barrier(0);                                       \
+    acc[3][3] = mfma(fw[3], fxa[3], acc[3][3]); __builtin_amdgcn_sched_barrier(0);                     \
+    L2_READ_X(fxa, 3, xaddr); __builtin_amdgcn_sched_barrier(0);                                       \
+    acc[3][4] = mfma(fw[3], fxa[4], acc[3][4]); __builtin_amdgcn_sched_barrier(0);                     \
+    L2_READ_X(fxa, 4, xaddr); L2_READ_W(3, waddr); __builtin_amdgcn_sched_barrier(0);                  \
+  } while (0)
+    L5_MFMAS(0); L2_READ_W(0, w1); __builtin_amdgcn_sched_barrier(0);
+    L5_MFMAS(1); L2_READ_W(1, w1); __builtin_amdgcn_sched_barrier(0);
+    if (pend_idx < NP) {
+      store_pending(pend_idx); store_pending(pend_idx + 1);
+      pend_idx += 2;
+      asm volatile("" : "+s"(pend_idx));
+      __builtin_amdgcn_sched_barrier(0);
+    }
+    if constexpr (RES != 0) {
+      if (kt == res_kt) { fetch_residual(res_tile); __builtin_amdgcn_sched_barrier(0); }
+    }
+    L5_MFMAS(2); L2_READ_W(2, w1); __builtin_amdgcn_sched_barrier(0);
+    L5_LAST(x1, w1);
+    const int nxt = cur == 2 ? 0 : cur + 1;
+    const uint32_t bn = static_cast<uint32_t>(nxt) * STG;
+    const uint32_t w0 = aW + bn, x0 = aX + bn;
+    L5_MFMAS(0);
+    L5_MFMAS(1);
+    LC_DRAIN();
+    LC_BARRIER();
+    __builtin_amdgcn_sched_barrier(0);
+    L2_READ_W(0, w0); L2_READ_W(1, w0); __builtin_amdgcn_sched_barrier(0);
+    L5_MFMAS(2); L2_READ_W(2, w0); __builtin_amdgcn_sched_barrier(0);
+    L5_LAST(x0, w0);
+#undef L5_MFMAS
+#undef L5_LAST
+    cur = nxt;
+    }
+  };
 
   for (int ti = 0; ti < my_tiles; ++ti) {
     bool second; int m0, n0;
@@ -688,32 +727,32 @@
 #pragma unroll
       for (int a = 0; a < 4; ++a)
 #pragma unroll
-        for (int b = 0; b < 4; ++b) acc[a][b] = lc_f32x4_t{0.f, 0.f, 0.f, 0.f};
-    }
-    if constexpr (RES == 1) { res_tile = ti + 1; res_kt = ti + 1 < my_tiles ? 4 : -1; }
-    if constexpr (RES == 2) { res_tile = ti; res_kt = 4; }
+        for (int b = 0; b < MF; ++b) acc[a][b] = lc_f32x4_t{0.f, 0.f, 0.f, 0.f};
+    }
+    if constexpr (RES == 1) { res_tile = ti + 1; res_kt = ti + 1 < my_tiles ? MF : -1; }
+    if constexpr (RES == 2) { res_tile = ti; res_kt = MF; }
     if constexpr (RES != 0) asm volatile("" : "+s"(res_kt));
     for (int kt = 0; kt < nk; ++kt) {
       asm volatile("" : "+s"(kt));
-      kstep(kt);
+      if constexpr (MF == 5) kstep5(kt);
+      else kstep(kt);
     }
 
     if (epi & EPI_BIAS) {
-      const uint32_t ab = lds_base + 3 * lcSTG + (ti & 1) * 1024 + (wn * 64 + fq * 4) * 4;
+      const uint32_t ab = lds_base + 3 * STG + (ti & 1) * 1024 + (wn * 64 + fq * 4) * 4;
       lc_f32x4_t bv[4];
 #pragma unroll
-      for (int a = 0; a < 4; ++a) asm volatile("ds_read_b128 %0, %1 offset:%2" : "=v"(bv[a]) : "v"(ab), "n"(a * 64));
-      asm volatile("s_waitcnt lgkmcnt(0)" : "+v"(bv[0]), "+v"(bv[1]), "+v"(bv[2]), "+v"(bv[3])::"memory");
+      for (int a = 0; a < 4; ++a) bv[a] = __builtin_bit_cast(lc_f32x4_t, lc_lds_read(ab + a * 64));
 #pragma unroll
       for (int a = 0; a < 4; ++a)
 #pragma unroll
-        for (int b = 0; b < 4; ++b) acc[a][b] += bv[a];
+        for (int b = 0; b < MF; ++b) acc[a][b] += bv[a];
     }
     if (epi & EPI_QUICKGELU) {
 #pragma unroll
       for (int a = 0; a < 4; ++a)
 #pragma unroll
-        for (int b = 0; b < 4; ++b)
+        for (int b = 0; b < MF; ++b)
 #pragma unroll
           for (int j = 0; j < 4; j += 2) {
             const lc_f32x2_t v = {acc[a][b][j], acc[a][b][j + 1]};
@@ -725,23 +764,23 @@
           }
     }
     if constexpr (RES == 2) {
-      asm volatile("s_waitcnt vmcnt(0)" : "+v"(pend[0]), "+v"(pend[1]), "+v"(pend[2]), "+v"(pend[3]), "+v"(pend[4]), "+v"(pend[5]), "+v"(pend[6]), "+v"(pend[7])::"memory");
-#pragma unroll
-      for (int b = 0; b < 4; ++b)
+      L2_PEND_WAIT();
+#pragma unroll
+      for (int b = 0; b < MF; ++b)
 #pragma unroll
         for (int pr = 0; pr < 2; ++pr) add_piece(b, pr, pend[2 * b + pr]);
     }
     if constexpr (RES == 1) {
       if (res_kt >= 0)
-        asm volatile("s_waitcnt vmcnt(0)" : "+v"(pend[0]), "+v"(pend[1]), "+v"(pend[2]), "+v"(pend[3]), "+v"(pend[4]), "+v"(pend[5]), "+v"(pend[6]), "+v"(pend[7])::"memory");
+        L2_PEND_WAIT();
     }
     __builtin_amdgcn_sched_barrier(0);
     {
       char* const obase = static_cast<char*>(out) + (static_cast<size_t>(m0) * N + n0) * 2;
       const uint32_t ldn = static_cast<uint32_t>(N) * 2;
-      const uint32_t off0 = static_cast<uint32_t>(wm * 64 + frow) * ldn + static_cast<uint32_t>(wn * 64 + (fq & 1) * 16 + (fq & 2) * 4) * 2;
-#pragma unroll
-      for (int b = 0; b < 4; ++b)
+      const uint32_t off0 = static_cast<uint32_t>(wm * 16 * MF + frow) * ldn + static_cast<uint32_t>(wn * 64 + (fq & 1) * 16 + (fq & 2) * 4) * 2;
+#pragma unroll
+      for (int b = 0; b < MF; ++b)
 #pragma unroll
         for (int pr = 0; pr < 2; ++pr) {
           uint32_t lo[2], hi[2];
@@ -766,26 +805,24 @@
           pend[2 * b + pr] = lc_u32x4_t{s0[0], s1[0], s0[1], s1[1]};
         }
       pend_base = obase; pend_off0 = off0; pend_ldn = ldn;
-      const bool full = m0 + lcBM <= M;
+      const bool full = m0 + BM <= M;
       if (full && ti + 1 < my_tiles && !(epi & 256)) {
         pend_idx = 0;
         asm volatile("" : "+s"(pend_idx));
       } else if (!(epi & 256)) {
 #pragma unroll
-        for (int b = 0; b < 4; ++b)
+        for (int b = 0; b < MF; ++b)
 #pragma unroll
           for (int pr = 0; pr < 2; ++pr)
-            if (m0 + wm * 64 + b * 16 + frow < M)
+            if (m0 + wm * 16 * MF + b * 16 + frow < M)
               *reinterpret_cast<lc_u32x4_t*>(obase + (off0 + static_cast<uint32_t>(b * 16) * ldn + pr * 64)) = pend[2 * b + pr];
       }
     }
   }
   asm volatile("s_waitcnt lgkmcnt(0)" ::: "memory");
-#undef L2_WAIT5
-#undef L2_WAIT1
-#undef L2_WAIT_ALLW
 #undef L2_READ_W
 #undef L2_READ_X
+#undef L2_PEND_WAIT
 }
 
 int gemm_lc_mode();
@@ -904,20 +941,16 @@
   };
 #define Q_READ2(dst, addr, off)                                                                                   \
   do {                                                                                                            \
-    asm volatile("ds_read_b128 %0, %1 offset:%2" : "=v"(dst[0]) : "v"(addr), "n"(off));                          \
-    asm volatile("ds_read_b128 %0, %1 offset:%2" : "=v"(dst[1]) : "v"((addr) ^ 64u), "n"(off));                  \
-  } while (0)
-#define Q_WAIT_ALL()                                                                                               \
-  asm volatile("s_waitcnt lgkmcnt(0)"                                                                             \
-               : "+v"(fw[0][0]), "+v"(fw[0][1]), "+v"(fw[1][0]), "+v"(fw[1][1]), "+v"(fw[2][0]), "+v"(fw[2][1]), "+v"(fw[3][0]), "+v"(fw[3][1]), \
-                 "+v"(fx[0][0]), "+v"(fx[0][1]), "+v"(fx[1][0]), "+v"(fx[1][1]), "+v"(fx[2][0]), "+v"(fx[2][1]), "+v"(fx[3][0]), "+v"(fx[3][1])::"memory")
+    (dst)[0] = lc_lds_read((addr) + (off));                                                                      \
+    (dst)[1] = lc_lds_read(((addr) ^ 64u) + (off));                                                              \
+  } while (0)
   int cur = 0;
-  __builtin_amdgcn_s_barrier();
+  LC_BARRIER();
   Q_READ2(fx[0], aX, 0); Q_READ2(fx[1], aX, 2048); Q_READ2(fx[2], aX, 4096); Q_READ2(fx[3], aX, 6144);
   Q_READ2(fw[0], aW, 0); Q_READ2(fw[1], aW, 2048); Q_READ2(fw[2], aW, 4096); Q_READ2(fw[3], aW, 6144);
   auto kstep = [&]() __attribute__((always_inline)) {
-    Q_WAIT_ALL();
-    __builtin_amdgcn_s_barrier();
+    LC_DRAIN();
+    LC_BARRIER();
     __builtin_amdgcn_sched_barrier(0);
     const int nxt = cur == 2 ? 0 : cur + 1;
     const uint32_t bn = static_cast<uint32_t>(nxt) * lcSTG;
@@ -1003,7 +1036,6 @@
   }
   asm volatile("s_waitcnt lgkmcnt(0)" ::: "memory");
 #undef Q_READ2
-#undef Q_WAIT_ALL
 }
 
 int launch_gemm_lc2q(const GemmProblem& g, int epi, hipStream_t st, hipEvent_t ev0, hipEvent_t ev1) {
@@ -1025,7 +1057,7 @@
          (epi & ~(EPI_BIAS | EPI_SCALE | 256)) == EPI_OUT_BF16;
 }
 
-static int lc_env_mode() { static const int m = []() { const char* e = getenv("CMH_GEMM_LC"); return e ? atoi(e) : 0; }(); return m; }
+static int lc_env_mode() { static const int m = []() { const char* e = getenv("CMH_GEMM_LC"); return e ? atoi(e) : 9; }(); return m; }
 static int g_lc_mode = -1;
 int gemm_lc_mode() { return g_lc_mode < 0 ? lc_env_mode() : g_lc_mode; }
 void gemm_lc_set_mode(int m) { g_lc_mode = m; }
@@ -1036,6 +1068,7 @@
     if (K < 512) return false;
     if (gemm_lc_mode() >= 5 && (epi & EPI_QUICKGELU)) return false;
     if (gemm_lc_mode() == 6 && (epi & EPI_RESIDUAL) && K / 64 > 16) return false;
+    if (gemm_lc_mode() == 9 && (epi & EPI_RESIDUAL)) return false;
   }
   if (!(epi & (EPI_OUT_BF16 | EPI_OUT_F16)) || ((epi & EPI_OUT_BF16) && (epi & EPI_OUT_F16))) return false;
   if (epi & ~(EPI_BIAS | EPI_QUICKGELU | EPI_RESIDUAL | EPI_RES_F16 | EPI_OUT_BF16 | EPI_OUT_F16 | 256)) return false;
@@ -1069,7 +1102,8 @@
   auto prob = [](const GemmProblem& g) {
     return LcProblem{static_cast<const char*>(g.A), static_cast<const char*>(g.W), g.bias, g.residual, g.out, g.m_dev, g.M, g.N, g.K};
   };
-  auto tiles_of = [](const GemmProblem& g) { return (g.N / lcBN) * ((g.M + lcBM - 1) / lcBM); };
+  const int bm = gemm_lc_mode() >= 8 ? 160 : lcBM;
+  auto tiles_of = [bm](const GemmProblem& g) { return (g.N / lcBN) * ((g.M + bm - 1) / bm); };
   const int cus = lc_cus();
   const int total = tiles_of(a) + (b ? tiles_of(*b) : 0);
   const int grid = total < cus ? ((total + 7) & ~7) : cus;
@@ -1077,10 +1111,15 @@
   if (gemm_lc_mode() >= 4) {
     const int res2 = !(epi & EPI_RESIDUAL) ? 0 : (gemm_lc_res_first(epi, a.K) ? 1 : 2);
     const bool f16 = (epi & EPI_OUT_F16) != 0;
+#define LC2_GO3(MF, G, R, F)                                                                                                  \
+  do {                                                                                                                       \
+    if (ev0) hipExtLaunchKernelGGL((gemm_lc2_kernel<MF, G, R, F>), dim3(grid), dim3(768), 0, st, ev0, ev1, 0, P0, P1, epi);  \
+    else hipLaunchKernelGGL((gemm_lc2_kernel<MF, G, R, F>), dim3(grid), dim3(768), 0, st, P0, P1, epi);                      \
+  } while (0)
 #define LC2_GO(G, R, F)                                                                                                       \
   do {                                                                                                                       \
-    if (ev0) hipExtLaunchKernelGGL((gemm_lc2_kernel<G, R, F>), dim3(grid), dim3(768), 0, st, ev0, ev1, 0, P0, P1, epi);      \
-    else hipLaunchKernelGGL((gemm_lc2_kernel<G, R, F>), dim3(grid), dim3(768), 0, st, P0, P1, epi);                          \
+    if (bm == 160) LC2_GO3(5, G, R, F);                                                                                      \
+    else LC2_GO3(4, G, R, F);                                                                                                \
   } while (0)
 #define LC2_GO_G(G)                                                                                                           \
   do {                                                                                                                       \
@@ -1092,6 +1131,7 @@
     if (b) LC2_GO_G(true); else LC2_GO_G(false);
 #undef LC2_GO_G
 #undef LC2_GO
+#undef LC2_GO3
     CMH_CHECK_LAUNCH("gemm (lc2)");
     return 0;
   }
@@ -1139,7 +1179,7 @@
 #endif
 
 extern "C" int cmh_set_gemm_lc(int32_t mode) {
-  CMH_CHECK_ARG(mode >= -1 && mode <= 7, "set_gemm_lc: mode %d (-1 environment, 0 off, 1 every eligible launch, 2 all but QuickGELU launches, 3 by cost model, 4 / 5 / 6 the 12-wave form for every block launch / without the QuickGELU ones / for QKV and out_proj only)", mode);
+  CMH_CHECK_ARG(mode >= -1 && mode <= 9, "set_gemm_lc: mode %d (-1 environment, 0 off, 1 every eligible launch, 2 all but QuickGELU launches, 3 by cost model, 4 / 5 / 6 the 12-wave form for every block launch / without the QuickGELU ones / for QKV and out_proj only, 7 its fp8 form, 8 its 160-row tile without the QuickGELU launches, 9 (default) the same for QKV only)", mode);
   cmh::gemm_lc_set_mode(mode);
   return CMH_OK;
 }
```

Result: no change. 60200, median of 6 (+0.4%).
